# gvanhoy/gr-liquiddsp

Measured on AMD Instinct MI355X. Metric: Msamples/s through flex_rx (QPSK r1/2 1024B), higher is better.
Workload: dtype f32; 1 GPU; flex_rx single stream per GPU, 20000000 samples (10 Msym), PSK4 r=1/2 (CONV_V27), 1024-B payload, CRC-24, 256-sample gaps, CFO/phase/delay + AWGN Es/N0=20 dB; frames_decoded_ok=1154, streams_per_gpu=1, blocks_in_flight=12, stage_events=none (fxrx_set_timing level 0), steps=1415, passes=independent captures (reset between passes), segments=256, repairs=0

## Files before the change

gr-liquiddsp_amd/csrc/fx_host.cpp:

```cpp
#include <hip/hip_runtime.h>
#include <algorithm>
#include <chrono>
#include <cmath>
#include <cstdio>
#include <cstdlib>
#include <cstring>
#include <memory>
#include <string>
#include <vector>
#include "../../include/fxrx.h"
#include "fx_device.h"
#include "fx_codec.hpp"
#include "fx_launch.h"
#include "fx_traffic.h"

namespace {

thread_local std::string g_err;
void set_err(const std::string &s) { g_err = s; }

#define HIP_OK(expr)                                                                          \
    do {                                                                                      \
        hipError_t e_ = (expr);                                                               \
        if (e_ != hipSuccess) {                                                               \
            set_err(std::string(#expr) + ": " + hipGetErrorString(e_));                       \
            return FXRX_ERR_HIP;                                                              \
        }                                                                                     \
    } while (0)

template <class T> struct DevBuf {
    T *p = nullptr; size_t cap = 0;
    int reserve(size_t n)
    {
        if (n <= cap) return 0;
        size_t nc = std::max(n, cap + cap / 2);
        if (p) (void)hipFree(p);
        p = nullptr; cap = 0;
        if (hipMalloc((void **)&p, nc * sizeof(T)) != hipSuccess) { set_err("hipMalloc failed"); return FXRX_ERR_HIP; }
        cap = nc; return 0;
    }
    ~DevBuf() { if (p) (void)hipFree(p); }
};
template <class T> struct PinBuf {
    T *p = nullptr; size_t cap = 0;
    int reserve(size_t n)
    {
        if (n <= cap) return 0;
        size_t nc = std::max(n, cap + cap / 2);
        if (p) (void)hipHostFree(p);
        p = nullptr; cap = 0;
        if (hipHostMalloc((void **)&p, nc * sizeof(T), hipHostMallocDefault) != hipSuccess) { set_err("hipHostMalloc failed"); return FXRX_ERR_HIP; }
        cap = nc; return 0;
    }
    int grow_keep(size_t n, size_t keep)
    {
        if (n <= cap) return 0;
        T *np = nullptr;
        if (hipHostMalloc((void **)&np, n * sizeof(T), hipHostMallocDefault) != hipSuccess) { set_err("hipHostMalloc failed"); return FXRX_ERR_HIP; }
        if (p) { std::memcpy(np, p, std::min(keep, cap) * sizeof(T)); (void)hipHostFree(p); }
        p = np; cap = n; return 0;
    }
    ~PinBuf() { if (p) (void)hipHostFree(p); }
};

constexpr size_t kUploadKernelMax = 64u << 20;
static bool pinned_device_ptr(const void *p, const void **dev, uintptr_t align_mask = 7u)
{
    if (!p || (reinterpret_cast<uintptr_t>(p) & align_mask)) return false;
    hipPointerAttribute_t a;
    if (hipPointerGetAttributes(&a, p) != hipSuccess) { (void)hipGetLastError(); return false; }
    if (a.type != hipMemoryTypeHost || !a.devicePointer) return false;
    *dev = a.devicePointer;
    return true;
}
inline unsigned iq_sample_bytes(int fmt) { return fmt == FXRX_IQ_FC32 ? 8u : fmt == FXRX_IQ_SC16 ? 4u : fmt == FXRX_IQ_SC8 ? 2u : 0u; }
constexpr unsigned kMaxDepth = 32;
constexpr unsigned kStateRing = kMaxDepth + 3;
constexpr uint32_t kRepairCap = 256;

struct StreamState {
    float2 *carry[3] = { nullptr, nullptr, nullptr };
    int64_t carry_cap = 0;
    int64_t total = 0;
    bool fresh_start = true;
    int64_t carry_bound = 0;
    unsigned noskip_left = 0;
};

struct IngestJob { unsigned stream = 0; const void *dev_src = nullptr; const void *host_src = nullptr; uint64_t n = 0; };

struct StreamSnap { int64_t tot0 = 0; bool fresh_start = true; int64_t carry_bound = 0; bool noskip = false; };

}

struct Out { fxrx_frame f; };

enum StageEv { kEvStart = 0, kEvWalk, kEvVerify, kEvChain, kEvPlan, kEvMf, kEvPll, kEvDec, kEvDone, kEvHandover, kEvCount };
enum DecList { kDecPlain = 0, kDecRs, kDecBatch, kDecFallback, kDecLists };

struct Slot {
    hipStream_t st = nullptr;
    hipEvent_t ev[kEvCount] = {};
    unsigned index = 0;
    bool busy = false;
    uint64_t seq = 0;
    std::vector<const float2 *> x; std::vector<uint64_t> n; std::vector<StreamSnap> snap;
    std::vector<DevBuf<float2>> d_in;
    std::vector<DevBuf<uint8_t>> d_raw;
    std::vector<IngestJob> ingest; int ingest_fmt = FXRX_IQ_FC32; float ingest_scale = 0.0f;
    PinBuf<uint8_t> hp_desc; DevBuf<uint8_t> d_desc;
    size_t NJ = 0, n_early = 0, n_late = 0, o_list = 0, o_streams = 0;
    DevBuf<FxWalkResult> d_wres; DevBuf<FxFrame> d_frames, d_chain; DevBuf<FxVerifyRun> d_runs;
    DevBuf<FxBlockHdr> d_hdr;
    DevBuf<uint32_t> d_chain_count, d_stream_base, d_mf_job, d_mf_c0, d_pll_list, d_dec_list, d_vb_items;
    DevBuf<uint32_t> d_plan_ws;
    DevBuf<uint32_t> d_req;
    DevBuf<uint32_t> d_prescan;
    uint32_t ps_jobs = 0, ps_words = 0, ps_hops = 0, ps_taken = 0, ps_fallback = 0;
    DevBuf<uint32_t> d_cstat;
    DevBuf<uint8_t> d_vb_vec;
    DevBuf<unsigned long long> d_vb_dw;
    DevBuf<uint32_t> d_vb_st;
    uint32_t vb_cap = 0, vb_blk = 0;
    uint64_t vb_dw_words = 0, vb_slots_alloc = 128;
    DevBuf<FxPayJob> d_pjobs; DevBuf<FxPayResult> d_pres;
    uint32_t run_cap = 0, chain_cap = 0, mf_cap = 0, frame_slots = 0;
    uint64_t sym_cap = 0, byte_cap = 0, dw_cap = 0, out_cap = 0;
    DevBuf<float2> d_symraw;
    DevBuf<uint8_t> d_hard, d_bufA, d_bufB, d_soft; DevBuf<unsigned long long> d_dw;
    PinBuf<FxBlockHdr> h_hdr; PinBuf<FxOutRec> h_recs; PinBuf<uint8_t> h_out, h_soft; PinBuf<float2> h_framesyms;
    PinBuf<float2> h_win, h_wintail; PinBuf<uint32_t> h_winflag; uint32_t win_reserved = 0;
    std::vector<Out> out;
    uint64_t n_syms = 0;
    fxrx_timing timing{};
    double host_submit_ms = 0.0;
    bool any_late = false;
    double dbg_submit_ms = 0.0, dbg_collect_ms = 0.0, dbg_gpu_start_ms = 0.0, dbg_gpu_done_ms = 0.0;
    bool force_noskip = false;
    int timing_level = 0;
    bool inchain = false;
    uint32_t kept_hops = 0, kept_cheap = 0, kept_vhops = 0, kept_vfail = 0, kept_repairs = 0;
    TailPlan tail;
    bool tail_launched = true;
    hipStream_t tail_st = nullptr;
    uint32_t list_cap() const { return chain_cap + 64 * FX_PLL_CLASSES; }
    uint32_t *dec_list(DecList which) const { return d_dec_list.p + (size_t)which * list_cap(); }
    FxBlockHdr *hdr_walk() const { return d_hdr.p; } FxBlockHdr *hdr_pay() const { return d_hdr.p + 1; }
    const FxWalkJob *jobs() const { return reinterpret_cast<const FxWalkJob *>(d_desc.p); } FxWalkJob *jobs_rw() const { return reinterpret_cast<FxWalkJob *>(d_desc.p); }
    const uint32_t *job_list() const { return reinterpret_cast<const uint32_t *>(d_desc.p + o_list); } const FxStreamDesc *streams() const { return reinterpret_cast<const FxStreamDesc *>(d_desc.p + o_streams); }
#ifdef FX_STAMPS
    FxPayResult *pres() const { return d_pres.p; }
#else
    FxPayResult *pres() const { return nullptr; }
#endif
};

struct fxrx_ctx_s {
    fxrx_config cfg{};
    FxTables *d_tables = nullptr;
    std::vector<StreamState> st;
    FxStreamState *d_state = nullptr; FxStreamState *h_state = nullptr;
    float taper = -1.0f;
    bool skip_seek = true;
    bool chain_slow = false;
    unsigned pll_waves = 1, dec_waves = 1;
    int n_cus = 256;
    uint64_t seq = 0;
    hipEvent_t prev_chain = nullptr;
    hipEvent_t carry_reader[3] = { nullptr, nullptr, nullptr };
    Traffic traffic;
    bool batch_viterbi = true;
    bool vb_clean = true;
    int inchain_repair = 1; unsigned inchain_left = 0;
    bool plan_fused = true;
    bool vb_early_tail = true;
    int timing_level = -1;
    hipEvent_t ref_event = nullptr; double ref_host_ms = 0.0;
    int debug_walk_twice = 0;
    int debug_stop_after = 0;
    uint32_t walk_per_cu = 2;
    hipStream_t st_chain = nullptr;
    uint32_t verify_per_cu = 4;
    uint32_t mf_per_cu = 0;
    uint32_t plan_grid = 0;
    uint32_t vb_debug = 0, vb_blk_force = 0;
    std::vector<std::unique_ptr<Slot>> slots; unsigned depth = 1, head = 0, tail = 0, inflight = 0;
    Slot *last = nullptr;
    uint64_t replays = 0, repairs_host = 0, late_decodes = 0;
    uint64_t late_reason[6] = {};
    uint64_t late_windows = 0;
    uint32_t detwin_reserve = 0;
    unsigned noskip_left = 0;
    unsigned debug_fail_submit = 0, debug_fail_collect = 0;
    uint64_t discarded = 0;
    size_t ingest_kernel_max = 1u << 20;
    float iq_scale[3] = { 1.0f, 1.0f / 32768.0f, 1.0f / 128.0f };
    unsigned tail_gang = 4;
    bool prescan = false; int prescan_hops = -1;
    std::vector<Slot *> gang;
    uint64_t gang_launches = 0, gang_members = 0;
};

namespace {

std::unique_ptr<FxTables> make_tables()
{
    const fx::HostTables &H = fx::host_tables();
    const fx::BlockCodes &B = fx::block_codes();
    std::unique_ptr<FxTables> t(new FxTables);
    std::memset(t.get(), 0, sizeof(FxTables));
    for (int i = 0; i < 512; i++) { t->tw[i] = make_float2(H.tw[i].re, H.tw[i].im); t->S[i] = make_float2(H.S[i].re, H.S[i].im); }
    for (int i = 0; i < 1024; i++) t->sc[i] = make_float2(H.sc[i].re, H.sc[i].im);
    for (int i = 0; i < FX_S_LEN; i++) t->s[i] = make_float2(H.s[i].re, H.s[i].im);
    for (int i = 0; i < FX_HDR_PILOTS; i++) t->pilots[i] = make_float2(H.pilots[i].re, H.pilots[i].im);
    for (int i = 0; i < FX_PN_LEN; i++) t->pn[i] = make_float2(H.pn[i].re, H.pn[i].im);
    fx::design_eq_init(t->eq0);
    std::memcpy(t->proto, H.proto, sizeof H.proto);
    t->s2sum = H.s2sum;
    {
        fx::cf td[512]; std::memset(td, 0, sizeof td);
        float e = 0.0f, mr = 0.0f, mi = 0.0f;
        const int nd = FX_S_LEN - 1;
        for (int k = 0; k < nd; k++) {
            td[k].re = H.s[k + 1].re * H.s[k].re + H.s[k + 1].im * H.s[k].im;
            td[k].im = H.s[k + 1].im * H.s[k].re - H.s[k + 1].re * H.s[k].im;
            mr += td[k].re; mi += td[k].im;
        }
        mr /= (float)nd; mi /= (float)nd;
        for (int k = 0; k < nd; k++) { td[k].re -= mr; td[k].im -= mi; e += td[k].re * td[k].re + td[k].im * td[k].im; }
        fx::cf TD[512]; fx::hfft::fft512(td, TD, H.tw);
        for (int i = 0; i < 512; i++) t->TD[i] = make_float2(TD[i].re, TD[i].im);
        t->td2sum = e;
    }
    for (size_t i = 0; i < H.perm54.size(); i++) t->perm54[i] = (uint16_t)H.perm54[i];
    for (size_t i = 0; i < H.perm27.size(); i++) t->perm27[i] = (uint16_t)H.perm27[i];
    std::memcpy(t->h84dec, B.h84_dec, 256); std::memcpy(t->h84enc, B.h84_enc, 16); std::memcpy(t->sdcol, B.sd_col, 64);
    std::memcpy(t->sd22col, B.sd22_col, 16); std::memcpy(t->sd39col, B.sd39_col, 32);
    std::memcpy(t->h74dec, B.h74_dec, 128); std::memcpy(t->h128dec, B.h128_dec, 4096);
    std::memcpy(t->golenc, B.gol_enc, sizeof B.gol_enc); std::memcpy(t->golerr, B.gol_err, sizeof B.gol_err);
    std::memcpy(t->rsexp, B.rs_exp, 512); std::memcpy(t->rslog, B.rs_log, 256);
    for (int d = 0; d < 16; d++) t->h74enc[d] = B.h74_enc[d];
    for (int d = 0; d < 256; d++) t->h128enc[d] = B.h128_enc[d];
    {
        const uint8_t *cols[3] = { B.sd22_col, B.sd39_col, B.sd_col };
        const unsigned ncol[3] = { 16, 32, 64 };
        for (int c = 0; c < 3; c++) for (unsigned j = 0; j < ncol[c]; j++) t->sdinv[c][cols[c][j]] = (uint8_t)(j + 1);
    }
    return t;
}

int upload_tables(fxrx_ctx_s *c)
{
    std::unique_ptr<FxTables> t = make_tables();
    HIP_OK(hipMalloc((void **)&c->d_tables, sizeof(FxTables)));
    HIP_OK(hipMemcpy(c->d_tables, t.get(), sizeof(FxTables), hipMemcpyHostToDevice));
    return 0;
}

inline uint32_t seg_frames_cap(uint64_t seg, bool detect) { return (uint32_t)std::min<uint64_t>(seg / (detect ? 256 : 600) + 8, 4000); }

int alloc_carry(StreamState &S, int64_t cap)
{
    for (auto &p : S.carry) {
        if (p) (void)hipFree(p);
        p = nullptr;
        if (hipMalloc((void **)&p, (size_t)cap * sizeof(float2)) != hipSuccess) { set_err("hipMalloc (carry buffer) failed"); return FXRX_ERR_HIP; }
    }
    S.carry_cap = cap;
    return 0;
}

bool is_block_fec(unsigned fec)
{
    return fec == FX_FEC_HAMMING74 || fec == FX_FEC_HAMMING84 || fec == FX_FEC_HAMMING128 || fec == FX_FEC_GOLAY2412 ||
           fec == FX_FEC_SECDED2216 || fec == FX_FEC_SECDED3932 || fec == FX_FEC_SECDED7264;
}

constexpr unsigned kDebugMaxN = 1u << 18;

template <class Launch>
int debug_decode(const char *who, const uint8_t *in, size_t in_bytes, size_t in_pad, void *out, size_t out_bytes, void *out2, size_t out2_bytes,
                        Launch launch)
{
    int nd = 0;
    if (hipGetDeviceCount(&nd) != hipSuccess || nd <= 0) { set_err(std::string(who) + ": no usable HIP device"); return FXRX_ERR_NODEVICE; }
    std::unique_ptr<FxTables> t = make_tables();
    FxTables *d_t = nullptr; uint8_t *d_in = nullptr, *d_out = nullptr, *d_out2 = nullptr;
    auto run = [&]() -> int {
        HIP_OK(hipMalloc((void **)&d_t, sizeof(FxTables)));
        HIP_OK(hipMalloc((void **)&d_in, in_bytes + in_pad));
        HIP_OK(hipMalloc((void **)&d_out, out_bytes));
        if (out2) HIP_OK(hipMalloc((void **)&d_out2, out2_bytes));
        HIP_OK(hipMemcpy(d_t, t.get(), sizeof(FxTables), hipMemcpyHostToDevice));
        HIP_OK(hipMemcpy(d_in, in, in_bytes, hipMemcpyHostToDevice));
        HIP_OK(launch(d_in, d_out, d_out2, d_t));
        HIP_OK(hipDeviceSynchronize());
        HIP_OK(hipMemcpy(out, d_out, out_bytes, hipMemcpyDeviceToHost));
        if (out2) HIP_OK(hipMemcpy(out2, d_out2, out2_bytes, hipMemcpyDeviceToHost));
        return 0;
    };
    const int rc = run();
    for (void *p : { (void *)d_t, (void *)d_in, (void *)d_out, (void *)d_out2 }) if (p) (void)hipFree(p);
    return rc;
}

}

__attribute__((constructor)) static void fxrx_default_hw_queues() { setenv("GPU_MAX_HW_QUEUES", "16", 0); }

extern "C" {

const char *fxrx_last_error(void) { return g_err.c_str(); }
void fxrx_set_error(const char *msg) { set_err(msg ? msg : ""); }
const char *fxrx_version(void) { return "fxrx 0.2 (gfx950)"; }
int fxrx_device_count(void) { int n = 0; if (hipGetDeviceCount(&n) != hipSuccess) return 0; return n; }
void *fxrx_pinned_alloc(size_t bytes)
{
    void *p = nullptr;
    if (hipHostMalloc(&p, bytes ? bytes : 1, hipHostMallocDefault) != hipSuccess) { set_err("fxrx_pinned_alloc: hipHostMalloc failed"); return nullptr; }
    return p;
}
void fxrx_pinned_free(void *p) { if (p) (void)hipHostFree(p); }

static int make_slot(fxrx_ctx_s *c)
{
    std::unique_ptr<Slot> s(new Slot);
    HIP_OK(hipStreamCreateWithFlags(&s->st, hipStreamNonBlocking));
    for (auto &e : s->ev) HIP_OK(hipEventCreate(&e));
    s->index = (unsigned)c->slots.size();
    if (s->h_hdr.reserve(1) || s->d_hdr.reserve(2)) return FXRX_ERR_HIP;
    std::memset(s->h_hdr.p, 0, sizeof(FxBlockHdr));
    HIP_OK(hipMemset(s->d_hdr.p, 0, 2 * sizeof(FxBlockHdr)));
    c->slots.push_back(std::move(s));
    return 0;
}

static int close_gang(fxrx_ctx_s *c);
static void sync_all(fxrx_ctx_s *c) { if (c->st_chain) (void)hipStreamSynchronize(c->st_chain); for (auto &s : c->slots) if (s->st) (void)hipStreamSynchronize(s->st); }

static double g_prof[8]; static unsigned long g_prof_n;
static const bool g_prof_on = std::getenv("FXRX_DEBUG_SUBMIT_PROFILE") != nullptr;
static inline double prof_now() { return std::chrono::duration<double, std::milli>(std::chrono::steady_clock::now().time_since_epoch()).count(); }
void fxrx_destroy(fxrx_ctx *c)
{
    if (!c) return;
    (void)hipSetDevice(c->cfg.device);
    (void)close_gang(c);
    sync_all(c);
    if (g_prof_on && g_prof_n) {
        std::fprintf(stderr, "[fxrx] submit profile over %lu blocks (ms per block): upload + bookkeeping %.4f, segments %.4f, memory + descriptors %.4f, front launches %.4f, back launches %.4f\n",
                     g_prof_n, g_prof[0] / g_prof_n, g_prof[1] / g_prof_n, g_prof[2] / g_prof_n, g_prof[3] / g_prof_n, g_prof[4] / g_prof_n);
        for (auto &v : g_prof) v = 0.0; g_prof_n = 0;
    }
    for (auto &s : c->slots) {
        for (auto e : s->ev) if (e) (void)hipEventDestroy(e);
        if (s->st) (void)hipStreamDestroy(s->st);
    }
    if (c->st_chain) { (void)hipStreamSynchronize(c->st_chain); (void)hipStreamDestroy(c->st_chain); }
    for (auto &S : c->st) for (auto &p : S.carry) if (p) (void)hipFree(p);
    if (c->d_tables) (void)hipFree(c->d_tables);
    if (c->d_state) (void)hipFree(c->d_state);
    if (c->h_state) (void)hipHostFree(c->h_state);
    delete c;
}

fxrx_ctx *fxrx_create(const fxrx_config *cfg)
{
    if (!cfg || cfg->n_streams == 0) { set_err("fxrx_create: bad config"); return nullptr; }
    if (cfg->mode == FXRX_MODE_DETECTOR && cfg->soft_header) { set_err("fxrx_create: soft_header needs flex_rx mode (FXRX_ERR_ARG)"); return nullptr; }
    if (cfg->soft_block && (cfg->mode == FXRX_MODE_DETECTOR || !cfg->soft_decision)) {
        set_err("fxrx_create: soft_block needs soft_decision and flex_rx mode (FXRX_ERR_ARG)"); return nullptr;
    }
    if (cfg->soft_chain && (cfg->mode == FXRX_MODE_DETECTOR || !cfg->soft_decision || !cfg->soft_block)) {
        set_err("fxrx_create: soft_chain needs soft_block, soft_decision and flex_rx mode (FXRX_ERR_ARG)"); return nullptr;
    }
    if (cfg->soft_rs && (cfg->mode == FXRX_MODE_DETECTOR || !cfg->soft_decision)) {
        set_err("fxrx_create: soft_rs needs soft_decision and flex_rx mode (FXRX_ERR_ARG)"); return nullptr;
    }
    int nd = 0;
    if (hipGetDeviceCount(&nd) != hipSuccess || nd <= 0 || cfg->device >= nd) {
        set_err("fxrx_create: no usable HIP device (this library has no CPU path)"); return nullptr;
    }
    if (hipSetDevice(cfg->device) != hipSuccess) { set_err("hipSetDevice failed"); return nullptr; }
    fxrx_ctx_s *c = new fxrx_ctx_s;
    auto fail = [&]() -> fxrx_ctx * { const std::string keep = g_err; fxrx_destroy(c); set_err(keep); return nullptr; };
    c->cfg = *cfg;
    if (c->cfg.threshold <= 0.0f) c->cfg.threshold = cfg->mode == FXRX_MODE_DETECTOR ? 0.45f : 0.5f;
    if (const char *e = std::getenv("FXRX_PLL_WAVES")) c->pll_waves = (unsigned)std::min(4, std::max(1, std::atoi(e)));
    if (const char *e = std::getenv("FXRX_DEC_WAVES")) c->dec_waves = (unsigned)std::min(8, std::max(1, std::atoi(e)));
    if (const char *e = std::getenv("FXRX_SKIP_SEEK")) c->skip_seek = std::atoi(e) != 0;
    if (const char *e = std::getenv("FXRX_TAPER")) c->taper = std::min(0.95f, (float)std::atof(e));
    if (const char *e = std::getenv("FXRX_CHAIN_SLOW")) c->chain_slow = std::atoi(e) != 0;
    if (const char *e = std::getenv("FXRX_BATCH_VITERBI")) c->batch_viterbi = std::atoi(e) != 0;
    if (const char *e = std::getenv("FXRX_VB_CLEAN")) c->vb_clean = std::atoi(e) != 0;
    if (const char *e = std::getenv("FXRX_INCHAIN_REPAIR")) c->inchain_repair = std::min(2, std::max(0, std::atoi(e)));
    if (const char *e = std::getenv("FXRX_PLAN_FUSED")) c->plan_fused = std::atoi(e) != 0;
    if (const char *e = std::getenv("FXRX_VB_EARLY_TAIL")) c->vb_early_tail = std::atoi(e) != 0;
    if (const char *e = std::getenv("FXRX_DEBUG_STOP_AFTER")) c->debug_stop_after = std::atoi(e);
    if (const char *e = std::getenv("FXRX_DEBUG_WALK_TWICE")) c->debug_walk_twice = std::atoi(e);
    if (const char *e = std::getenv("FXRX_TIMING")) c->timing_level = std::min(2, std::max(0, std::atoi(e)));
    if (const char *e = std::getenv("FXRX_WALK_PER_CU")) c->walk_per_cu = (uint32_t)std::min(8, std::max(1, std::atoi(e)));
    if (const char *e = std::getenv("FXRX_VERIFY_PER_CU")) c->verify_per_cu = (uint32_t)std::min(64, std::max(1, std::atoi(e)));
    if (const char *e = std::getenv("FXRX_MF_PER_CU")) c->mf_per_cu = (uint32_t)std::min(64, std::max(0, std::atoi(e)));
    if (const char *e = std::getenv("FXRX_INGEST_KERNEL_MAX")) c->ingest_kernel_max = (size_t)std::max<long long>(0, std::atoll(e));
    if (const char *e = std::getenv("FXRX_PLAN_GRID")) c->plan_grid = (uint32_t)std::min(256, std::max(0, std::atoi(e)));
    if (const char *e = std::getenv("FXRX_DETWIN_RESERVE")) c->detwin_reserve = (uint32_t)std::max(0, std::atoi(e));
    if (const char *e = std::getenv("FXRX_VB_DEBUG")) c->vb_debug = (uint32_t)std::atoi(e);
    if (const char *e = std::getenv("FXRX_PRESCAN")) c->prescan = std::atoi(e) != 0;
    if (const char *e = std::getenv("FXRX_PRESCAN_HOPS")) c->prescan_hops = std::min<int>(FX_PRESCAN_MAX_HOPS, std::max(0, std::atoi(e)));
    if (const char *e = std::getenv("FXRX_TAIL_GANG")) c->tail_gang = (unsigned)std::min(FX_GANG_MAX, std::max(1, std::atoi(e)));
    if (const char *e = std::getenv("FXRX_VB_BLK")) if (std::atoi(e) > 0) c->vb_blk_force = (uint32_t)std::min(4096, std::max(128, (std::atoi(e) + 63) / 64 * 64));
    hipDeviceProp_t prop;
    if (hipGetDeviceProperties(&prop, cfg->device) == hipSuccess) c->n_cus = prop.multiProcessorCount;
    if (const char *e = std::getenv("FXRX_DEBUG_CUS")) c->n_cus = std::min(c->n_cus, std::max(1, std::atoi(e)));
    if (upload_tables(c) != 0) return fail();
    const unsigned NS = cfg->n_streams;
    c->st.resize(NS);
    int64_t cap0 = std::max<int64_t>(1 << 15, std::min<int64_t>(1 << 18, (int64_t)(1 << 24) / (int64_t)NS));
    if (const char *e = std::getenv("FXRX_CARRY_SAMPLES")) cap0 = std::max<int64_t>(1024, std::atoll(e));
    for (auto &S : c->st) if (alloc_carry(S, cap0) != 0) return fail();
    if (hipMalloc((void **)&c->d_state, sizeof(FxStreamState) * kStateRing * NS) != hipSuccess ||
        hipHostMalloc((void **)&c->h_state, sizeof(FxStreamState) * kStateRing * NS, hipHostMallocDefault) != hipSuccess) { set_err("fxrx_create: state ring allocation failed"); return fail(); }
    if (hipMemset(c->d_state, 0, sizeof(FxStreamState) * kStateRing * NS) != hipSuccess) { set_err("hipMemset failed"); return fail(); }
    std::memset(c->h_state, 0, sizeof(FxStreamState) * kStateRing * NS);
    for (unsigned i = 0; i < 2; i++) if (make_slot(c) != 0) return fail();
    return c;
}

void fxrx_reset(fxrx_ctx *c)
{
    if (!c) return;
    for (auto &S : c->st) { S.total = 0; S.fresh_start = true; S.carry_bound = 0; }
}

int fxrx_set_depth(fxrx_ctx *c, unsigned int depth)
{
    if (!c || depth == 0 || depth > kMaxDepth) return FXRX_ERR_ARG;
    HIP_OK(hipSetDevice(c->cfg.device));
    { const int r = close_gang(c); if (r) return r; }
    if (c->inflight) { set_err("fxrx_set_depth: blocks in flight"); return FXRX_ERR_STATE; }
    while (c->slots.size() < depth + 1) if (make_slot(c) != 0) return FXRX_ERR_HIP;
    c->depth = depth; c->head = c->tail = 0; c->last = nullptr;
    return 0;
}

int fxrx_debug_block_times(const fxrx_ctx *c, double out[4])
{
    if (!c || !c->last || !out) return FXRX_ERR_ARG;
    out[0] = c->last->dbg_submit_ms; out[1] = c->last->dbg_gpu_start_ms; out[2] = c->last->dbg_gpu_done_ms; out[3] = c->last->dbg_collect_ms;
    return 0;
}

int fxrx_set_timing(fxrx_ctx *c, int level)
{
    if (!c || level < -1 || level > 2) return FXRX_ERR_ARG;
    c->timing_level = level;
    if (!c->gang.empty()) { HIP_OK(hipSetDevice(c->cfg.device)); return close_gang(c); }
    return 0;
}

void *fxrx_stream(const fxrx_ctx *c) { return (c && !c->slots.empty()) ? (void *)c->slots[0]->st : nullptr; }

int fxrx_last_timing(const fxrx_ctx *c, fxrx_timing *t) { if (!c || !t || !c->last) return FXRX_ERR_ARG; *t = c->last->timing; return 0; }

const void *fxrx_device_framesyms(const fxrx_ctx *c, uint64_t *n)
{
    if (!c || !c->last) return nullptr;
    if (n) *n = c->last->n_syms;
    return c->last->n_syms ? c->last->d_symraw.p : nullptr;
}

enum WalkForm { kWalkList, kWalkRequests, kWalkRequestsInChain };
static inline hipError_t launch_walk(const fxrx_ctx_s *c, const Slot &sl, hipStream_t st, const uint32_t *list, unsigned njobs, WalkForm form = kWalkList)
{
    return fx_launch_walk(c->cfg.mode == FXRX_MODE_DETECTOR ? FX_MODE_DETECT : FX_MODE_FLEXRX, c->cfg.equalizer ? 1 : 0, c->cfg.soft_header ? 1 : 0, njobs, st, sl.jobs(), list, sl.d_wres.p, sl.d_frames.p, sl.d_runs.p,
                          sl.run_cap, sl.hdr_walk(), c->d_tables, form == kWalkList ? 0 : 1, (uint32_t)sl.NJ, form == kWalkRequestsInChain ? &sl.hdr_walk()->n_repair_req : nullptr, form == kWalkRequestsInChain ? (uint32_t)(2 * sl.NJ + 16) : 0u);
}
static inline hipError_t launch_seekverify(const fxrx_ctx_s *c, const Slot &sl, hipStream_t st, unsigned grid, uint32_t phase)
{
    return fx_launch_seekverify(grid, st, sl.d_runs.p, sl.run_cap, sl.jobs(), sl.d_wres.p, sl.d_frames.p, sl.hdr_walk(), c->d_tables, phase);
}
enum ChainForm { kStitch, kStitchQueue, kStitchPass1, kStitchPass2 };
static inline hipError_t launch_chainfast(const fxrx_ctx_s *c, const Slot &sl, hipStream_t st, ChainForm form)
{
    const bool queue = form == kStitchQueue || form == kStitchPass1;
    return fx_launch_chainfast(c->cfg.n_streams, st, sl.streams(), sl.jobs(), sl.d_wres.p, sl.d_frames.p, sl.d_chain.p, sl.d_chain_count.p, sl.hdr_walk(), form == kStitch && c->chain_slow ? 1u : 0u,
                               queue ? sl.jobs_rw() : nullptr, queue ? sl.d_req.p : nullptr, form >= kStitchPass1 ? sl.d_cstat.p : nullptr, form == kStitchPass1 ? 1u : form == kStitchPass2 ? 2u : 0u);
}
static inline int soft_level(const fxrx_config &cfg) { return cfg.soft_decision ? (cfg.soft_block ? (cfg.soft_chain ? 3 : 2) : 1) : 0; }
static inline hipError_t launch_paydec(const fxrx_ctx_s *c, const Slot &sl, hipStream_t st, DecList which, unsigned first_wave, unsigned n_waves, unsigned waves_per_wg)
{
    return fx_launch_paydec(which == kDecRs ? 1 : 0, which == kDecFallback ? 0 : soft_level(c->cfg), c->cfg.soft_rs ? 1 : 0, first_wave, n_waves, waves_per_wg, st, sl.d_pjobs.p, sl.dec_list(which), sl.hdr_pay(), sl.d_hard.p, sl.d_bufA.p, sl.d_bufB.p,
                            sl.d_soft.p, sl.d_dw.p, sl.h_out.p, sl.h_recs.p, sl.pres(), c->d_tables, which == kDecFallback ? sl.h_hdr.p : nullptr);
}
static inline hipError_t launch_decoders(const fxrx_ctx_s *c, const Slot &sl, hipStream_t st, unsigned first_plain, unsigned n_plain, unsigned n_rs)
{
    const hipError_t e = launch_paydec(c, sl, st, kDecPlain, first_plain, n_plain, c->dec_waves);
    return e != hipSuccess ? e : launch_paydec(c, sl, st, kDecRs, 0u, n_rs, 1u);
}
static inline hipError_t launch_trellis(const fxrx_ctx_s *c, const Slot &sl, hipStream_t st, unsigned n_items, int packed, int with_fix, unsigned n_fin, unsigned fb_waves)
{
    hipError_t e = fx_launch_vbitems(0, n_items, st, sl.d_pjobs.p, sl.d_vb_items.p, sl.vb_cap, sl.hdr_pay(), sl.d_bufA.p, sl.d_bufB.p, sl.d_vb_dw.p, sl.d_vb_vec.p, sl.d_vb_st.p, c->vb_debug, packed, with_fix);
    if (e == hipSuccess) e = fx_launch_vbfinish(0, n_fin, st, sl.d_pjobs.p, sl.dec_list(kDecBatch), sl.hdr_pay(), sl.d_bufA.p, sl.d_bufB.p, sl.d_vb_dw.p, sl.d_vb_vec.p, sl.d_vb_st.p, sl.dec_list(kDecFallback),
                                                sl.list_cap(), sl.h_out.p, sl.h_recs.p, sl.h_hdr.p, sl.tail.vb_early ? 1 : 0);
    return e != hipSuccess ? e : launch_paydec(c, sl, st, kDecFallback, 0u, fb_waves, 1u);
}
static inline hipError_t launch_detwin(const fxrx_ctx_s *c, const Slot &sl, uint32_t first, uint32_t last, bool late)
{
    return fx_launch_detwin(sl.st, std::min<unsigned>(std::max<unsigned>(last - first, 1u), 4u * (unsigned)c->n_cus), sl.streams(), c->cfg.n_streams, sl.d_stream_base.p, sl.d_pjobs.p, sl.hdr_pay(), first, last,
                            sl.h_win.p, sl.h_wintail.p, sl.h_winflag.p, late ? 0 : 1, late ? 1 : 0);
}
static void mark_noskip(fxrx_ctx_s *c, const Slot &sl, const std::vector<uint32_t> &req)
{
    const FxWalkJob *hj = reinterpret_cast<const FxWalkJob *>(sl.hp_desc.p);
    for (uint32_t r : req) if ((r & 0x80000000u) && (r & 0x7fffffffu) < sl.NJ) c->st[hj[r & 0x7fffffffu].stream].noskip_left = 32;
}

enum { kChainFast = 0, kChainFull = 1, kChainDone = 2 };
static int enqueue_back(fxrx_ctx_s *c, Slot &sl, int chain_mode, hipStream_t chain_st = nullptr, bool may_defer = false);

static int enqueue_block(fxrx_ctx_s *c, Slot &sl, bool may_defer = false)
{
    const unsigned NS = c->cfg.n_streams;
    const bool detect = c->cfg.mode == FXRX_MODE_DETECTOR;
    const uint64_t b = sl.seq;
    hipStream_t st = sl.st;
    const double tp0 = g_prof_on ? prof_now() : 0.0;

    uint32_t ps_K = 0;
    if (c->prescan && !detect) {
        if (c->prescan_hops >= 0) ps_K = (uint32_t)c->prescan_hops;
        else {
            ps_K = c->traffic.frames ? (uint32_t)std::min<uint64_t>(128, std::max<uint64_t>(16, c->traffic.samples / c->traffic.frames / FX_HOP + 2)) : 64u;
            ps_K = (ps_K + FX_PRESCAN_CHUNK - 1) / FX_PRESCAN_CHUNK * FX_PRESCAN_CHUNK;
        }
    }

    uint64_t seg = c->cfg.segment_len;
    if (seg == 0) {
        uint64_t tot = 0;
        for (unsigned s = 0; s < NS; s++) tot += sl.n[s];
        const uint64_t slots = (uint64_t)c->n_cus * c->walk_per_cu;
        if (c->depth > 1 && !detect) seg = tot / std::max<uint64_t>(std::max<uint64_t>(1, c->n_cus), std::min<uint64_t>(slots, 6 * slots / c->depth));
        else if (tot / slots < 131072) seg = tot / (slots - slots / 16);
        else seg = std::max<uint64_t>(tot / (4 * slots), 65536);
        seg = std::max<uint64_t>(seg, 32768); seg = std::min<uint64_t>(seg, 1u << 20);
    }
    seg = std::max<uint64_t>(seg, 4096);
    float taper = c->taper;
    if (taper < 0.0f) {
        uint64_t tot = 0;
        for (unsigned s = 0; s < NS; s++) tot += sl.n[s];
        taper = (detect && tot / seg > 4ull * (uint64_t)c->n_cus) ? 0.75f : 0.0f;
    }
    std::vector<FxWalkJob> jobs; std::vector<uint32_t> early, late; std::vector<FxStreamDesc> sds(NS);
    uint32_t frame_slots = 0, chain_slots = 0; uint64_t n_total = 0, carry_total = 0;
    for (unsigned s = 0; s < NS; s++) {
        StreamState &S = c->st[s]; const StreamSnap &sn = sl.snap[s];
        const int64_t ns = (int64_t)sl.n[s];
        const bool cont = !sn.fresh_start;
        FxStreamDesc &sd = sds[s];
        sd.x = sl.x[s]; sd.xa_end = cont ? S.carry[b % 3] + S.carry_cap : nullptr; sd.n = ns;
        sd.first_job = (uint32_t)jobs.size();
        sd.state_in = cont ? c->d_state + ((b + kStateRing - 1) % kStateRing) * NS + s : nullptr;
        sd.state_out = c->d_state + (b % kStateRing) * NS + s;
        sd.state_out_host = c->h_state + (b % kStateRing) * NS + s;
        sd.carry_out_end = S.carry[(b + 1) % 3] + S.carry_cap; sd.carry_cap = S.carry_cap;
        sd.abs_base = sn.tot0;
        int64_t p = 0; bool first = true;
        const int64_t seg0 = cont ? (int64_t)std::min<uint64_t>(seg, 8192) : (int64_t)seg;
        const int64_t p_t = cont ? std::min<int64_t>(ns, seg0) : 0;
        const int64_t k_t = taper > 0.0f ? std::max<int64_t>(1, ((ns - p_t) + (int64_t)seg / 2) / (int64_t)seg) : 0;
        int64_t i_t = 0;
        while (first || p < ns) {
            FxWalkJob j{};
            j.x = sd.x; j.xa_end = sd.xa_end; j.n = ns; j.start = p;
            j.stop = std::min<int64_t>(ns, p + (first ? seg0 : (int64_t)seg));
            if (ns - j.stop < (int64_t)seg / 2) j.stop = ns;
            if (k_t > 1 && p >= p_t) {
                const double u = (double)(i_t + 1) / (double)k_t;
                const int64_t e = p_t + (int64_t)((double)(ns - p_t) * (u * (1.0 + taper) - taper * u * u));
                j.stop = (i_t + 1 >= k_t) ? ns : std::min<int64_t>(ns, std::max<int64_t>(p + 4096, e & ~(int64_t)255));
                i_t++;
            }
            j.fresh = 1u; j.floor = p;
            j.mode = detect ? FX_MODE_DETECT : FX_MODE_FLEXRX;
            j.handoff = j.stop < ns ? 1u : 0u;
            j.prelock = first ? 0u : 1u;
            j.frame_base = frame_slots; j.max_frames = seg_frames_cap((uint64_t)(j.stop - j.start) + (first && cont ? (uint64_t)sn.carry_bound : 0u), detect);
            frame_slots += j.max_frames;
            j.threshold = c->cfg.threshold;
            j.no_skip = (detect || !c->skip_seek || sl.force_noskip || sn.noskip) ? 1u : 0u;
            j.state_in = (first && cont) ? sd.state_in : nullptr;
            j.stream = s; j.verify_per = c->traffic.verify_per; j.eq = (!detect && c->cfg.equalizer) ? 1u : 0u;
            (first && cont ? late : early).push_back((uint32_t)jobs.size());
            jobs.push_back(j);
            p = j.stop; first = false;
            if (p >= ns) break;
        }
        sd.n_jobs = (uint32_t)jobs.size() - sd.first_job;
        sd.chain_base = chain_slots; sd.chain_cap = (uint32_t)((uint64_t)(ns + (cont ? sn.carry_bound : 0)) / (detect ? 256u : 600u) + 8u);
        chain_slots += sd.chain_cap;
        n_total += (uint64_t)ns; carry_total += cont ? (uint64_t)sn.carry_bound : 0u;
    }
    for (unsigned s = 0; s < NS; s++) { sds[s].repair_base = frame_slots; sds[s].repair_cap = kRepairCap; frame_slots += kRepairCap; }
    if (taper > 0.0f)
        std::stable_sort(early.begin(), early.end(), [&](uint32_t a, uint32_t b2) { return jobs[a].stop - jobs[a].start > jobs[b2].stop - jobs[b2].start; });
    const size_t NJ = jobs.size();
    sl.NJ = NJ; sl.n_early = early.size(); sl.n_late = late.size(); sl.any_late = !late.empty();
    sl.frame_slots = frame_slots; sl.chain_cap = chain_slots;
    sl.run_cap = (uint32_t)std::min<uint64_t>((n_total + carry_total) / FX_HOP + 2 * NJ + 1024, 0x7fffffffu);
    const uint64_t span = n_total + carry_total;
    sl.sym_cap = span / 2 + 8ull * chain_slots + 64;
    sl.byte_cap = (span / 2) * 3 / 4 + 48ull * chain_slots + 64;
    sl.dw_cap = detect ? 0 : (span / 2) * 6 + 200ull * chain_slots + 64;
    sl.out_cap = (span / 2) * 3 / 4 + 16ull * chain_slots + 64;
    sl.mf_cap = (uint32_t)std::min<uint64_t>(span / 2 / 1024 + chain_slots + 16, 0x7fffffffu);
    {
        const uint64_t want_items = 64ull * 4ull * (uint64_t)c->n_cus * 6ull;
        sl.vb_blk = (detect || c->cfg.soft_decision || !c->batch_viterbi) ? 0u
                  : (uint32_t)std::min<uint64_t>(4096, std::max<uint64_t>(192, ((c->traffic.vb_steps / want_items + 63) / 64) * 64));
    }
    if (sl.vb_blk && c->vb_blk_force) sl.vb_blk = c->vb_blk_force;
    {
        const uint64_t steps_cap = std::min<uint64_t>(std::max<uint64_t>(span + span / 2, c->traffic.vb_steps + c->traffic.vb_steps / 4), 4 * span);
        sl.vb_cap = sl.vb_blk ? (uint32_t)((steps_cap / sl.vb_blk + 2048 + 127) & ~127ull) : 128u;
        sl.vb_dw_words = sl.vb_blk ? std::max<uint64_t>((uint64_t)sl.vb_cap * sl.vb_blk, steps_cap + 2176ull * 4096ull) : 0;
        sl.vb_slots_alloc = sl.vb_blk ? std::max<uint64_t>(sl.vb_cap, steps_cap / 192 + 2176) : 128;
    }
    if (sl.sym_cap >= (1ull << 32) || sl.dw_cap >= (1ull << 32)) { set_err("fxrx_submit: batch too large for 32-bit arena offsets"); return FXRX_ERR_ARG; }

    const double tp1 = g_prof_on ? prof_now() : 0.0;
    auto up16 = [](size_t v) { return (v + 15) & ~(size_t)15; };
    const size_t o_list = up16(NJ * sizeof(FxWalkJob)), o_streams = o_list + up16(2 * NJ * sizeof(uint32_t)), desc_bytes = o_streams + up16(NS * sizeof(FxStreamDesc));
    sl.o_list = o_list; sl.o_streams = o_streams;
    std::vector<uint32_t> spec;
    if (ps_K) for (uint32_t ji : early) if (jobs[ji].prelock && jobs[ji].mode == FX_MODE_FLEXRX) spec.push_back(ji);
    sl.ps_jobs = (uint32_t)spec.size(); sl.ps_hops = ps_K; sl.ps_words = (ps_K + FX_PRESCAN_CHUNK - 1) / FX_PRESCAN_CHUNK; sl.ps_taken = sl.ps_fallback = 0;
    if (!spec.empty()) {
        if (sl.d_prescan.reserve(spec.size() * sl.ps_words)) return FXRX_ERR_HIP;
        for (size_t i = 0; i < spec.size(); i++) {
            FxWalkJob &j = jobs[spec[i]];
            j.prescan = sl.d_prescan.p + i * sl.ps_words; j.prescan_words = sl.ps_words;
            j.prescan_hops = fx_prescan_valid_hops(j.start, j.stop, j.n, ps_K);
        }
    }
    if (sl.hp_desc.reserve(desc_bytes) || sl.d_desc.reserve(desc_bytes) || sl.d_wres.reserve(NJ + NS) || sl.d_frames.reserve(frame_slots) ||
        sl.d_runs.reserve(sl.run_cap) || sl.d_req.reserve(2 * NJ + 16) || sl.d_cstat.reserve(NS) || sl.d_chain.reserve(chain_slots) || sl.d_chain_count.reserve(NS) || sl.d_stream_base.reserve(NS + 1) ||
        sl.d_pjobs.reserve(chain_slots) || sl.h_recs.reserve(chain_slots) || sl.d_mf_job.reserve(sl.mf_cap) || sl.d_mf_c0.reserve(sl.mf_cap) ||
        sl.d_pll_list.reserve(sl.list_cap()) || sl.d_dec_list.reserve(kDecLists * (size_t)sl.list_cap())) return FXRX_ERR_HIP;
    if (!detect && (sl.d_symraw.reserve(sl.sym_cap) || sl.d_hard.reserve(sl.sym_cap + 64) ||
                    sl.d_bufA.reserve(sl.byte_cap + 256) || sl.d_bufB.reserve(sl.byte_cap + 256) || sl.d_dw.reserve(sl.dw_cap) || sl.h_out.reserve(sl.out_cap))) return FXRX_ERR_HIP;
    if (!detect && c->cfg.want_framesyms && sl.h_framesyms.reserve(sl.sym_cap)) return FXRX_ERR_HIP;
    if (detect && c->cfg.want_framesyms) {
        sl.win_reserved = c->detwin_reserve ? std::min(chain_slots, c->detwin_reserve) : with_margin(c->traffic.frames, chain_slots);
        if (sl.h_win.reserve((size_t)sl.win_reserved * FX_NFFT) || sl.h_wintail.reserve(2 * (size_t)NS * FX_NFFT) || sl.h_winflag.reserve(1)) return FXRX_ERR_HIP;
        *sl.h_winflag.p = 0u;
    }
    if (!sl.d_plan_ws.p) {
        if (sl.d_plan_ws.reserve(fx_plan_ws_words())) return FXRX_ERR_HIP;
        HIP_OK(hipMemsetAsync(sl.d_plan_ws.p, 0, fx_plan_ws_words() * sizeof(uint32_t), st));
    }
    if (sl.d_vb_items.reserve(2 * (size_t)sl.vb_slots_alloc) ||
        (sl.vb_blk && (sl.d_vb_vec.reserve(128 * (size_t)sl.vb_slots_alloc) || sl.d_vb_dw.reserve((size_t)sl.vb_dw_words) || sl.d_vb_st.reserve(sl.vb_slots_alloc)))) return FXRX_ERR_HIP;
    if (!detect && c->cfg.soft_decision && (sl.d_soft.reserve(8 * sl.byte_cap) || (c->cfg.want_framesyms && sl.h_soft.reserve(8 * sl.byte_cap)))) return FXRX_ERR_HIP;
#ifdef FX_STAMPS
    if (!detect && sl.d_pres.reserve(chain_slots)) return FXRX_ERR_HIP;
#endif
    std::memcpy(sl.hp_desc.p, jobs.data(), NJ * sizeof(FxWalkJob));
    uint32_t *hl = reinterpret_cast<uint32_t *>(sl.hp_desc.p + o_list);
    if (!early.empty()) std::memcpy(hl, early.data(), early.size() * sizeof(uint32_t));
    if (!late.empty()) std::memcpy(hl + early.size(), late.data(), late.size() * sizeof(uint32_t));
    if (!spec.empty()) std::memcpy(hl + NJ, spec.data(), spec.size() * sizeof(uint32_t));
    std::memcpy(sl.hp_desc.p + o_streams, sds.data(), NS * sizeof(FxStreamDesc));
    const uint32_t *d_list = sl.job_list();

    const double tp2 = g_prof_on ? prof_now() : 0.0;
    if (!sl.ingest.empty()) {
        std::vector<IngestJob> todo; todo.swap(sl.ingest);
        const size_t bytes = iq_sample_bytes(sl.ingest_fmt);
        for (const IngestJob &j : todo) {
            const void *src = j.dev_src;
            if (!src) { HIP_OK(hipMemcpyAsync(sl.d_raw[j.stream].p, j.host_src, j.n * bytes, hipMemcpyHostToDevice, st)); src = sl.d_raw[j.stream].p; }
            HIP_OK(fx_launch_ingest(st, sl.ingest_fmt, src, sl.d_in[j.stream].p, (size_t)j.n, sl.ingest_scale, (unsigned)c->n_cus));
        }
    }
    HIP_OK(fx_launch_upload(st, sl.hp_desc.p, sl.d_desc.p, desc_bytes, (unsigned)c->n_cus));
    const int tl = c->timing_level >= 0 ? c->timing_level : (c->depth > 1 ? 0 : 2);
    sl.timing_level = tl;
    if (c->debug_walk_twice > 0) HIP_OK(fx_launch_prescan(st, (unsigned)spec.size(), sl.ps_words, sl.jobs(), d_list + NJ, c->d_tables));
    for (int rep = 0; rep < c->debug_walk_twice; rep++) HIP_OK(launch_walk(c, sl, st, d_list, (unsigned)early.size()));
    if (tl >= 2) HIP_OK(hipEventRecord(sl.ev[kEvStart], st));
    if (c->debug_walk_twice <= 0) HIP_OK(fx_launch_prescan(st, (unsigned)spec.size(), sl.ps_words, sl.jobs(), d_list + NJ, c->d_tables));
    HIP_OK(launch_walk(c, sl, st, d_list, (unsigned)early.size()));
    const bool verify = !detect && c->skip_seek && !sl.force_noskip;
    hipStream_t cst = st;
    if (!late.empty()) {
        if (verify) {
            HIP_OK(fx_launch_copy_u32(st, &sl.hdr_walk()->n_runs, &sl.hdr_walk()->runs_done));
            HIP_OK(launch_seekverify(c, sl, st, c->verify_per_cu * (unsigned)c->n_cus, 0u));
        }
        if (!c->st_chain) {
            int lo = 0, hi = 0;
            HIP_OK(hipDeviceGetStreamPriorityRange(&lo, &hi));
            HIP_OK(hipStreamCreateWithPriority(&c->st_chain, hipStreamNonBlocking, hi));
        }
        HIP_OK(hipEventRecord(sl.ev[kEvHandover], st));
        cst = c->st_chain;
        HIP_OK(hipStreamWaitEvent(cst, sl.ev[kEvHandover], 0));
        if (c->prev_chain) HIP_OK(hipStreamWaitEvent(cst, c->prev_chain, 0));
        HIP_OK(launch_walk(c, sl, cst, d_list + early.size(), (unsigned)late.size()));
    }
    if (tl >= 2) HIP_OK(hipEventRecord(sl.ev[kEvWalk], cst));
    if (verify)
        HIP_OK(launch_seekverify(c, sl, cst, late.empty() ? c->verify_per_cu * (unsigned)c->n_cus : (unsigned)std::min<size_t>((size_t)c->verify_per_cu * (size_t)c->n_cus, std::max<size_t>(64, 16 * late.size())), 1u));
    if (tl >= 2) HIP_OK(hipEventRecord(sl.ev[kEvVerify], cst));
    if (late.empty() && c->prev_chain) HIP_OK(hipStreamWaitEvent(cst, c->prev_chain, 0));
    if (c->carry_reader[(b + 1) % 3]) HIP_OK(hipStreamWaitEvent(cst, c->carry_reader[(b + 1) % 3], 0));
    const double tp3 = g_prof_on ? prof_now() : 0.0;
    const int rb = enqueue_back(c, sl, kChainFast, cst, may_defer);
    if (g_prof_on) { const double tp4 = prof_now(); g_prof[1] += tp1 - tp0; g_prof[2] += tp2 - tp1; g_prof[3] += tp3 - tp2; g_prof[4] += tp4 - tp3; g_prof_n++; }
    return rb;
}

static FxVbpreMember vbpre_member(Slot &sl, uint32_t first_wave, uint32_t n_waves)
{
    return FxVbpreMember{ sl.d_pjobs.p, sl.dec_list(kDecBatch), sl.hdr_pay(), sl.d_hard.p, sl.d_bufA.p, sl.d_bufB.p, sl.h_out.p, sl.h_recs.p, sl.h_hdr.p, first_wave, n_waves };
}
static int launch_tails(fxrx_ctx_s *c, Slot *const *m, unsigned n)
{
    hipStream_t st = m[n - 1]->st;
    for (unsigned i = 0; i + 1 < n; i++) HIP_OK(hipStreamWaitEvent(st, m[i]->ev[kEvMf], 0));
    auto done = [&]() -> int {
        for (unsigned i = 0; i < n; i++) { HIP_OK(hipEventRecord(m[i]->ev[kEvDone], st)); m[i]->tail_launched = true; m[i]->tail_st = st; }
        if (n > 1) { c->gang_launches++; c->gang_members += n; }
        return 0;
    };
    {
        FxPllGang g; unsigned waves[FX_GANG_MAX]; g.n = n;
        for (unsigned i = 0; i < n; i++) { const Slot &sl = *m[i]; g.m[i] = FxPllMember{ sl.d_pjobs.p, sl.d_pll_list.p, sl.hdr_pay(), sl.d_symraw.p, sl.d_symraw.p, sl.d_hard.p, sl.h_recs.p }; waves[i] = sl.tail.pll_waves; }
        HIP_OK(fx_launch_paypll(&g, waves, c->pll_waves, st, c->d_tables));
    }
    for (unsigned i = 0; i < n; i++) if (m[i]->timing_level >= 1) HIP_OK(hipEventRecord(m[i]->ev[kEvPll], st));
    if (c->debug_stop_after == 6) return done();
    for (unsigned i = 0; i < n; i++) {
        Slot &sl = *m[i];
        if (c->cfg.soft_decision) {
            HIP_OK(fx_launch_softdemod(sl.tail.mf_grid, st, sl.d_pjobs.p, sl.d_mf_job.p, sl.d_mf_c0.p, sl.hdr_pay(), sl.d_symraw.p, sl.d_hard.p, sl.d_soft.p, c->d_tables));
            if (c->cfg.want_framesyms) HIP_OK(hipMemcpyAsync(sl.h_soft.p, sl.d_soft.p, 8 * sl.byte_cap, hipMemcpyDeviceToHost, st));
        }
        HIP_OK(launch_decoders(c, sl, st, 0u, sl.tail.plain, sl.tail.rs));
    }
    {
        FxVbpreGang g; g.n = n;
        for (unsigned i = 0; i < n; i++) g.m[i] = vbpre_member(*m[i], 0u, m[i]->vb_blk ? m[i]->tail.vb_pre : 0u);
        HIP_OK(fx_launch_vbpre(&g, st, c->d_tables, c->vb_clean ? 1 : 0, c->vb_early_tail && c->vb_clean ? 1 : 0));
    }
    for (unsigned i = 0; i < n; i++) {
        Slot &sl = *m[i];
        if (sl.vb_blk) HIP_OK(launch_trellis(c, sl, st, sl.tail.vb_items, sl.tail.vb_packed, sl.tail.with_fix, sl.tail.vb_fin, sl.tail.fb));
        if (sl.timing_level >= 2) HIP_OK(hipEventRecord(sl.ev[kEvDec], st));
        if (c->cfg.want_framesyms) HIP_OK(fx_launch_symcopy(2u * (unsigned)c->n_cus, st, sl.hdr_pay(), sl.d_symraw.p, sl.h_framesyms.p));
    }
    return done();
}

static int close_gang(fxrx_ctx_s *c)
{
    if (c->gang.empty()) return 0;
    if (c->gang.size() > FX_GANG_MAX) { set_err("open gang larger than FX_GANG_MAX (internal error)"); return FXRX_ERR_STATE; }
    Slot *m[FX_GANG_MAX]; unsigned n = 0;
    for (Slot *s : c->gang) m[n++] = s;
    c->gang.clear();
    return launch_tails(c, m, n);
}

static int enqueue_back(fxrx_ctx_s *c, Slot &sl, int chain_mode, hipStream_t chain_st, bool may_defer)
{
    const unsigned NS = c->cfg.n_streams; const bool detect = c->cfg.mode == FXRX_MODE_DETECTOR;
    const uint64_t b = sl.seq; const uint32_t chain_slots = sl.chain_cap; hipStream_t st = sl.st;
    sl.tail_launched = true; sl.tail_st = st;
    if (chain_mode == kChainFull)
        HIP_OK(fx_launch_chain(detect ? FX_MODE_DETECT : FX_MODE_FLEXRX, c->cfg.equalizer ? 1 : 0, c->cfg.soft_header ? 1 : 0, NS, st, sl.streams(), sl.jobs(), (uint32_t)sl.NJ, sl.d_wres.p, sl.d_frames.p, sl.d_chain.p,
                               sl.d_chain_count.p, sl.d_runs.p, sl.run_cap, sl.hdr_walk(), c->chain_slow ? 1u : 0u, c->d_tables));
    else if (chain_mode == kChainFast) {
        hipStream_t cs = chain_st ? chain_st : st;
        sl.inchain = !c->chain_slow && (c->inchain_repair == 2 || (c->inchain_repair == 1 && c->inchain_left > 0));
        if (c->inchain_left) c->inchain_left--;
        if (!sl.inchain) HIP_OK(launch_chainfast(c, sl, cs, kStitch));
        else {
            HIP_OK(launch_chainfast(c, sl, cs, kStitchPass1));
            HIP_OK(launch_walk(c, sl, cs, sl.d_req.p, (unsigned)std::min<size_t>(2 * sl.NJ, 64), kWalkRequestsInChain));
            HIP_OK(launch_chainfast(c, sl, cs, kStitchPass2));
        }
    }
    HIP_OK(hipEventRecord(sl.ev[kEvChain], chain_mode == kChainFast && chain_st ? chain_st : st));
    if (chain_mode == kChainFast && chain_st && chain_st != st) HIP_OK(hipStreamWaitEvent(st, sl.ev[kEvChain], 0));
    c->prev_chain = sl.ev[kEvChain];
    {
        FxPlanArgs a;
        a.streams = sl.streams(); a.nstreams = NS; a.detect = detect ? 1u : 0u; a.eq = c->cfg.equalizer ? 1u : 0u; a.vb_blk = sl.vb_blk;
        a.chain = sl.d_chain.p; a.chain_count = sl.d_chain_count.p; a.stream_base = sl.d_stream_base.p;
        a.pjobs = sl.d_pjobs.p; a.recs = sl.h_recs.p;
        a.mf_job = sl.d_mf_job.p; a.mf_c0 = sl.d_mf_c0.p; a.mf_cap = sl.mf_cap;
        a.pll_list = sl.d_pll_list.p; a.dec_list = sl.dec_list(kDecPlain); a.list_cap = sl.list_cap();
        a.vb_items = sl.d_vb_items.p; a.vb_cap = sl.vb_cap;
        a.hdr = sl.hdr_walk(); a.hdr_pay = sl.hdr_pay(); a.hdr_host = sl.h_hdr.p; a.ws = sl.d_plan_ws.p;
        HIP_OK(fx_launch_plan(st, c->plan_grid ? c->plan_grid : (unsigned)std::min<uint64_t>(64, c->traffic.frames / 2048 + 1), c->plan_fused ? 1 : 0, a));
    }
    const int tl = sl.timing_level;
    if (tl >= 2) HIP_OK(hipEventRecord(sl.ev[kEvPlan], st));
    if (c->debug_stop_after == 4) { c->carry_reader[b % 3] = nullptr; HIP_OK(hipEventRecord(sl.ev[kEvDone], st)); return 0; }
    if (!detect) {
        const TailPlan plan = plan_tail(c->traffic, TailCaps{ chain_slots, sl.mf_cap, sl.vb_cap, sl.vb_blk }, TailKnobs{ c->depth, c->n_cus, c->mf_per_cu, c->vb_debug, c->vb_early_tail, c->vb_clean });
        HIP_OK(fx_launch_paymf(plan.mf_grid, c->cfg.equalizer ? 1 : 0, st, sl.d_pjobs.p, sl.d_mf_job.p, sl.d_mf_c0.p, sl.hdr_pay(), sl.d_chain.p, sl.d_symraw.p, c->d_tables));
        HIP_OK(hipEventRecord(sl.ev[kEvMf], st));
        c->carry_reader[b % 3] = sl.ev[kEvMf];
        if (c->debug_stop_after == 5) { HIP_OK(hipEventRecord(sl.ev[kEvDone], st)); return 0; }
        sl.tail = plan;
        if (sl.vb_blk && c->traffic.trellis_left) c->traffic.trellis_left--;
        sl.timing.trellis_launched = plan.vb_fin ? 1 : 0;
        unsigned ahead = 0;
        for (unsigned k = 0; k < c->inflight; k++) ahead += c->slots[(c->tail + k) % (c->depth + 1)]->tail_launched ? 1u : 0u;
        const unsigned G = c->tail_gang;
        if (G >= 2 && may_defer && c->depth >= 4 && c->traffic.seen && !c->debug_stop_after && tl <= 1 && ahead >= G) {
            sl.tail_launched = false; sl.tail_st = nullptr;
            c->gang.push_back(&sl);
            return c->gang.size() >= G ? close_gang(c) : 0;
        }
        { const int r = close_gang(c); if (r) return r; }
        Slot *one = &sl;
        return launch_tails(c, &one, 1u);
    } else {
        if (c->cfg.want_framesyms) HIP_OK(launch_detwin(c, sl, 0u, sl.win_reserved, false));
        HIP_OK(hipEventRecord(sl.ev[kEvMf], st));
        if (tl >= 1) HIP_OK(hipEventRecord(sl.ev[kEvPll], st));
        if (tl >= 2) HIP_OK(hipEventRecord(sl.ev[kEvDec], st));
        c->carry_reader[b % 3] = sl.ev[kEvMf];
    }
    HIP_OK(hipEventRecord(sl.ev[kEvDone], st));
    return 0;
}

static int prepare_ingest(fxrx_ctx_s *c, Slot &sl, const void *const *iq, const uint64_t *n_samples, int on_device, int fmt)
{
    const unsigned NS = c->cfg.n_streams;
    const size_t bytes = iq_sample_bytes(fmt);
    sl.ingest.clear();
    for (unsigned s = 0; s < NS; s++)
        if (n_samples[s] && (!iq[s] || (reinterpret_cast<uintptr_t>(iq[s]) & (bytes - 1)))) {
            set_err("fxrx_submit_fmt: integer IQ must be aligned to its sample size (sc16: 4 bytes, sc8: 2 bytes)"); return FXRX_ERR_ARG;
        }
    if (sl.d_in.size() < NS) sl.d_in.resize(NS);
    if (sl.d_raw.size() < NS) sl.d_raw.resize(NS);
    std::vector<IngestJob> jobs;
    for (unsigned s = 0; s < NS; s++) {
        const uint64_t nn = n_samples[s];
        if (sl.d_in[s].reserve(nn + 1)) return FXRX_ERR_HIP;
        if (!nn) continue;
        IngestJob j; j.stream = s; j.n = nn;
        if (on_device) j.dev_src = iq[s];
        else if (!(nn * bytes <= c->ingest_kernel_max && pinned_device_ptr(iq[s], &j.dev_src, 0u))) {
            j.dev_src = nullptr; j.host_src = iq[s];
            if (sl.d_raw[s].reserve(nn * bytes + 16)) return FXRX_ERR_HIP;
        }
        jobs.push_back(j);
    }
    sl.ingest.swap(jobs); sl.ingest_fmt = fmt; sl.ingest_scale = c->iq_scale[fmt];
    return 0;
}

static int submit_block(fxrx_ctx *c, const void *const *iq, const uint64_t *n_samples, int on_device, int fmt)
{
    if (!c || !iq || !n_samples) { set_err("fxrx_submit: null argument"); return FXRX_ERR_ARG; }
    if (iq_sample_bytes(fmt) == 0) { set_err("fxrx_submit_fmt: unknown IQ format"); return FXRX_ERR_ARG; }
    if (c->inflight >= c->depth) { set_err("fxrx_submit: pipeline full, call fxrx_collect first"); return FXRX_ERR_STATE; }
    HIP_OK(hipSetDevice(c->cfg.device));
    const auto t_enter = std::chrono::steady_clock::now();
    const unsigned NS = c->cfg.n_streams;
    const unsigned nslots = c->depth + 1;
    Slot &sl = *c->slots[c->head];
    sl.ingest.clear();
    if (fmt != FXRX_IQ_FC32) { const int r = prepare_ingest(c, sl, iq, n_samples, on_device, fmt); if (r) return r; }
    sl.out.clear(); sl.timing = fxrx_timing{};
    sl.kept_hops = sl.kept_cheap = sl.kept_vhops = sl.kept_vfail = sl.kept_repairs = 0;
    const unsigned noskip_before = c->noskip_left;
    sl.force_noskip = c->noskip_left > 0; if (c->noskip_left) c->noskip_left--;
    sl.seq = c->seq;
    sl.x.assign(NS, nullptr); sl.n.assign(n_samples, n_samples + NS); sl.snap.assign(NS, StreamSnap{});
    if (sl.d_in.size() < NS) sl.d_in.resize(NS);
    struct Undo { fxrx_ctx_s *c; std::vector<StreamState> st; unsigned noskip; bool armed = true;
                  ~Undo() { if (armed) { c->st = st; c->noskip_left = noskip; } } } undo{ c, c->st, noskip_before };
    uint64_t total_new = 0;
    for (unsigned s = 0; s < NS; s++) {
        StreamState &S = c->st[s];
        const uint64_t nn = n_samples[s];
        total_new += nn;
        if (fmt != FXRX_IQ_FC32) sl.x[s] = sl.d_in[s].p;
        else if (on_device) sl.x[s] = (const float2 *)iq[s];
        else {
            if (sl.d_in[s].reserve(nn + 1)) return FXRX_ERR_HIP;
            if (nn) {
                const void *dsrc = nullptr;
                if (nn * sizeof(float2) <= kUploadKernelMax && pinned_device_ptr(iq[s], &dsrc)) HIP_OK(fx_launch_upload(sl.st, dsrc, sl.d_in[s].p, nn * sizeof(float2), (unsigned)c->n_cus));
                else HIP_OK(hipMemcpyAsync(sl.d_in[s].p, iq[s], nn * sizeof(float2), hipMemcpyHostToDevice, sl.st));
            }
            sl.x[s] = sl.d_in[s].p;
        }
        sl.snap[s].tot0 = S.total; sl.snap[s].fresh_start = S.fresh_start; sl.snap[s].carry_bound = S.fresh_start ? 0 : S.carry_bound;
        sl.snap[s].noskip = S.noskip_left > 0; if (S.noskip_left) S.noskip_left--;
        S.total += (int64_t)nn; S.fresh_start = false;
        S.carry_bound = std::min<int64_t>(S.carry_cap, sl.snap[s].carry_bound + (int64_t)nn);
    }
    if (c->timing_level >= 2 && !c->ref_event) {
        if (hipEventCreate(&c->ref_event) == hipSuccess) { (void)hipEventRecord(c->ref_event, sl.st); (void)hipEventSynchronize(c->ref_event); c->ref_host_ms = std::chrono::duration<double, std::milli>(std::chrono::steady_clock::now().time_since_epoch()).count(); }
    }
    sl.dbg_submit_ms = std::chrono::duration<double, std::milli>(std::chrono::steady_clock::now().time_since_epoch()).count() - c->ref_host_ms;
    sl.timing.samples = total_new;
    if (c->debug_fail_submit) { c->debug_fail_submit--; set_err("fxrx_submit: injected failure (fxrx_debug_fail)"); return FXRX_ERR_STATE; }
    if (g_prof_on) g_prof[0] += prof_now() - std::chrono::duration<double, std::milli>(t_enter.time_since_epoch()).count();
    int r = enqueue_block(c, sl,  true);
    if (r) return r;
    undo.armed = false;
    c->seq++;
    sl.busy = true;
    c->head = (c->head + 1) % nslots; c->inflight++;
    sl.host_submit_ms = std::chrono::duration<double, std::milli>(std::chrono::steady_clock::now() - t_enter).count();
    return 0;
}

int fxrx_submit(fxrx_ctx *c, const void *const *iq, const uint64_t *n_samples, int on_device) { return submit_block(c, iq, n_samples, on_device, FXRX_IQ_FC32); }
int fxrx_submit_fmt(fxrx_ctx *c, const void *const *iq, const uint64_t *n_samples, int on_device, int fmt) { return submit_block(c, iq, n_samples, on_device, fmt); }

unsigned int fxrx_iq_sample_bytes(int fmt) { return iq_sample_bytes(fmt); }

int fxrx_set_iq_scale(fxrx_ctx *c, int fmt, float scale)
{
    if (!c || (fmt != FXRX_IQ_SC16 && fmt != FXRX_IQ_SC8) || !std::isfinite(scale) || !(scale > 0.0f)) { set_err("fxrx_set_iq_scale: bad argument"); return FXRX_ERR_ARG; }
    c->iq_scale[fmt] = scale;
    return 0;
}

int fxrx_iq_convert_host(int fmt, float scale, const void *in, uint64_t n_samples, float *out_re_im)
{
    if (iq_sample_bytes(fmt) == 0 || (n_samples && (!in || !out_re_im))) { set_err("fxrx_iq_convert_host: bad argument"); return FXRX_ERR_ARG; }
    const uint64_t nc = 2 * n_samples;
    if (fmt == FXRX_IQ_FC32) { if (nc) std::memcpy(out_re_im, in, nc * sizeof(float)); }
    else if (fmt == FXRX_IQ_SC16) { const int16_t *q = static_cast<const int16_t *>(in); for (uint64_t i = 0; i < nc; i++) out_re_im[i] = (float)q[i] * scale; }
    else { const int8_t *q = static_cast<const int8_t *>(in); for (uint64_t i = 0; i < nc; i++) out_re_im[i] = (float)q[i] * scale; }
    return 0;
}

static int repair_rounds(fxrx_ctx_s *c, Slot &sl)
{
    if (c->chain_slow) return 1;
    hipStream_t st = sl.st; FxBlockHdr *hdr = sl.hdr_walk();
    for (int round = 0; round < 64; round++) {
        HIP_OK(hipMemsetAsync(hdr, 0, sizeof(FxBlockHdr), st));
        HIP_OK(launch_chainfast(c, sl, st, kStitchQueue));
        FxBlockHdr hh;
        HIP_OK(hipMemcpyAsync(&hh, hdr, sizeof hh, hipMemcpyDeviceToHost, st));
        HIP_OK(hipStreamSynchronize(st));
        if (std::getenv("FXRX_DEBUG_ROUNDS")) std::fprintf(stderr, "[fxrx] repair round %d: flags %x requests %u\n", round, hh.flags, hh.n_repair_req);
        if (!(hh.flags & FX_BLK_NEEDS_REPAIR)) return 0;
        if ((hh.flags & FX_BLK_NEEDS_SLOW) || hh.n_repair_req == 0 || hh.n_repair_req > 2 * sl.NJ) break;
        {
            std::vector<uint32_t> req(hh.n_repair_req);
            HIP_OK(hipMemcpyAsync(req.data(), sl.d_req.p, req.size() * sizeof(uint32_t), hipMemcpyDeviceToHost, st));
            HIP_OK(hipStreamSynchronize(st));
            mark_noskip(c, sl, req);
        }
        HIP_OK(hipMemsetAsync(hdr, 0, sizeof(FxBlockHdr), st));
        HIP_OK(launch_walk(c, sl, st, sl.d_req.p, hh.n_repair_req, kWalkRequests));
        HIP_OK(hipMemcpyAsync(&hh, hdr, sizeof hh, hipMemcpyDeviceToHost, st));
        HIP_OK(hipStreamSynchronize(st));
        sl.kept_hops += hh.hops; sl.kept_cheap += hh.hops_cheap; sl.kept_repairs += hh.walk_jobs_run ? hh.walk_jobs_run : 0;
    }
    HIP_OK(hipMemsetAsync(hdr, 0, sizeof(FxBlockHdr), st));
    return 1;
}

static int repair_and_replay(fxrx_ctx_s *c, Slot &sl)
{
    const unsigned NS = c->cfg.n_streams;
    const unsigned nslots = c->depth + 1;
    unsigned n_dep = 0;
    for (unsigned k = 1; k < c->inflight; k++) {
        const Slot &nx = *c->slots[(c->tail + k) % nslots];
        bool dep = false;
        for (unsigned s = 0; s < NS; s++) dep = dep || !nx.snap[s].fresh_start;
        if (!dep) break;
        n_dep++;
    }
    const hipEvent_t newest_chain = c->prev_chain;
    bool carry_moved = false;
    { const int r = close_gang(c); if (r) return r; }
    for (int round = 0; round < 6; round++) {
        HIP_OK(hipStreamSynchronize(sl.st));
        for (unsigned k = 1; k <= n_dep; k++) {
            const Slot &nx = *c->slots[(c->tail + k) % nslots];
            HIP_OK(hipStreamSynchronize(nx.st));
            if (nx.tail_st && nx.tail_st != nx.st) HIP_OK(hipStreamSynchronize(nx.tail_st));
        }
        const uint32_t flags = sl.h_hdr.p->flags;
        if (std::getenv("FXRX_DEBUG_ROUNDS")) std::fprintf(stderr, "[fxrx] block %llu at collect: flags %x verify_failures %u (pass %d)\n", (unsigned long long)sl.seq, flags, sl.h_hdr.p->verify_failures, round);
        if (flags & FX_BLK_NEEDS_REPAIR) {
            c->repairs_host++; c->inchain_left = 16;
            const FxBlockHdr &h0 = *sl.h_hdr.p;
            sl.kept_hops += h0.hops; sl.kept_cheap += h0.hops_cheap; sl.kept_vhops += h0.verify_hops; sl.kept_vfail += h0.verify_failures;
            sl.ps_taken += h0.ps_taken; sl.ps_fallback += h0.ps_fallback;
            if (!sl.force_noskip && c->cfg.mode != FXRX_MODE_DETECTOR && c->skip_seek && h0.verify_failures > std::max<uint32_t>(16u, (uint32_t)sl.NJ / 8u)) {
                sl.force_noskip = true; c->noskip_left = 32;
                if (enqueue_block(c, sl)) return FXRX_ERR_HIP;
            } else {
                const int rr = repair_rounds(c, sl);
                if (rr < 0 || enqueue_back(c, sl, rr == 0 ? kChainDone : kChainFull)) return FXRX_ERR_HIP;
            }
            continue;
        }
        if (!(flags & FX_BLK_CARRY_OVERFLOW)) break;
        const uint64_t b = sl.seq;
        FxStreamState *hs = c->h_state + (b % kStateRing) * NS, *ds = c->d_state + (b % kStateRing) * NS;
        for (auto &o : c->slots) if (o->busy) HIP_OK(hipStreamSynchronize(o->st));
        carry_moved = true;
        for (unsigned s = 0; s < NS; s++) {
            if (!hs[s].overflow) continue;
            StreamState &S = c->st[s];
            const int64_t keep = hs[s].carry_len, old_cap = S.carry_cap;
            float2 *old[3] = { S.carry[0], S.carry[1], S.carry[2] };
            S.carry[0] = S.carry[1] = S.carry[2] = nullptr;
            int64_t cap = std::max<int64_t>(2 * old_cap, 2 * keep); cap = (cap + 4095) & ~(int64_t)4095;
            if (alloc_carry(S, cap)) return FXRX_ERR_HIP;
            const int64_t nb = (int64_t)sl.n[s], from = nb - keep;
            float2 *dst = S.carry[(b + 1) % 3] + cap - keep;
            if (from < 0) HIP_OK(hipMemcpy(dst, old[b % 3] + old_cap + from, (size_t)(-from) * sizeof(float2), hipMemcpyDeviceToDevice));
            const int64_t n_new = std::min<int64_t>(keep, nb);
            if (n_new > 0) HIP_OK(hipMemcpy(dst + (keep - n_new), sl.x[s] + (nb - n_new), (size_t)n_new * sizeof(float2), hipMemcpyDeviceToDevice));
            for (auto p : old) if (p) (void)hipFree(p);
            hs[s].overflow = 0; hs[s].invalid = 0;
            HIP_OK(hipMemcpy(ds + s, hs + s, sizeof(FxStreamState), hipMemcpyHostToDevice));
        }
        sl.h_hdr.p->flags &= ~(uint32_t)FX_BLK_CARRY_OVERFLOW;
        c->replays++;
        break;
    }
    if (sl.h_hdr.p->flags & (FX_BLK_NEEDS_REPAIR | FX_BLK_CARRY_OVERFLOW)) { set_err("fxrx_collect: block could not be repaired"); return FXRX_ERR_STATE; }
    if (sl.h_hdr.p->flags & FX_BLK_CHAIN_FULL) { set_err("fxrx_collect: chain table overflow (internal sizing error)"); return FXRX_ERR_STATE; }
    c->prev_chain = sl.ev[kEvChain];
    const unsigned n_replay = carry_moved ? c->inflight - 1 : n_dep;
    for (unsigned k = 1; k <= n_replay; k++) {
        Slot &nx = *c->slots[(c->tail + k) % nslots];
        for (unsigned s = 0; s < NS; s++) if (!nx.snap[s].fresh_start) nx.snap[s].carry_bound = c->st[s].carry_cap;
        int r = enqueue_block(c, nx);
        if (r) return r;
    }
    if (n_replay + 1 < c->inflight) c->prev_chain = newest_chain;
    for (auto &S : c->st) S.carry_bound = S.carry_cap;
    return 0;
}

static int finish_decode(fxrx_ctx_s *c, Slot &sl)
{
    FxBlockHdr *hdr_pay = sl.hdr_pay();
    auto fetch_fb = [&]() -> int { uint32_t nfb = 0; HIP_OK(hipMemcpy(&nfb, &hdr_pay->n_vb_fallback, sizeof nfb, hipMemcpyDeviceToHost)); sl.h_hdr.p->n_vb_fallback = nfb; sl.h_hdr.p->vb_ticket = 0; return 0; };
    if (sl.vb_blk && sl.h_hdr.p->vb_ticket && fetch_fb()) return FXRX_ERR_HIP;
    FxBlockHdr h = *sl.h_hdr.p; h.vb_dirty = *(volatile const uint32_t *)&sl.h_hdr.p->vb_dirty;
    TailPlan &p = sl.tail;
    const LateWork w = late_work(p, h, sl.vb_blk);
    if (!w.any()) return 0;
    HIP_OK(launch_decoders(c, sl, sl.st, p.plain, w.more_plain ? h.n_dec_plain - p.plain : 0u, w.more_rs ? h.n_dec_rs : 0u));
    if (w.more_batch() || w.late_trellis) {
        HIP_OK(hipMemsetAsync(&hdr_pay->n_vb_fallback, 0, sizeof(uint32_t), sl.st));
        if (w.more_batch()) {
            FxVbpreGang g; g.n = 1; g.m[0] = vbpre_member(sl, 0u, h.n_dec_batch);
            HIP_OK(fx_launch_vbpre(&g, sl.st, c->d_tables, c->vb_clean ? 1 : 0, p.vb_early ? 1 : 0));
        }
        HIP_OK(launch_trellis(c, sl, sl.st, h.n_vb_items, 1, 1, h.n_dec_batch, kFallbackWaves));
        p.vb_pre = p.vb_fin = h.n_dec_batch; p.vb_items = h.n_vb_items; p.fb = kFallbackWaves;
        HIP_OK(hipStreamSynchronize(sl.st));
        if (fetch_fb()) return FXRX_ERR_HIP;
    }
    const uint32_t n_fb = *(volatile const uint32_t *)&sl.h_hdr.p->n_vb_fallback;
    if (sl.vb_blk && n_fb > p.fb) {
        HIP_OK(launch_paydec(c, sl, sl.st, kDecFallback, p.fb, n_fb - p.fb, c->dec_waves));
        p.fb = n_fb;
    }
    HIP_OK(hipStreamSynchronize(sl.st));
    p.plain = std::max(p.plain, h.n_dec_plain); if (w.more_rs) p.rs = h.n_dec_rs;
    c->late_decodes++;
    w.count(c->late_reason);
    return 0;
}

static int finish_windows(fxrx_ctx_s *c, Slot &sl)
{
    if (*(volatile const uint32_t *)sl.h_winflag.p) { set_err("fxrx_collect: more than two detections of a stream start in its carried tail (internal sizing error)"); return FXRX_ERR_STATE; }
    const uint32_t n = sl.h_hdr.p->n_frames;
    if (n <= sl.win_reserved) return 0;
    { const int r = sl.h_win.grow_keep((size_t)n * FX_NFFT, (size_t)sl.win_reserved * FX_NFFT); if (r) return r; }
    HIP_OK(launch_detwin(c, sl, sl.win_reserved, n, true));
    HIP_OK(hipStreamSynchronize(sl.st));
    c->late_windows++;
    return 0;
}

static void discard_inflight(fxrx_ctx_s *c)
{
    const std::string keep = g_err;
    (void)close_gang(c);
    sync_all(c);
    const unsigned nslots = c->depth + 1;
// ... 291 lines not shown
```

gr-liquiddsp_amd/csrc/fx_kernels.hip:

```cpp
#include <hip/hip_runtime.h>
#include <algorithm>
#include "fx_device.h"
#include "fx_launch.h"
#include "fx_vbclean.h"
#include "fx_rsgmd.h"

#define HALF         256

template <int WW> struct WalkLdsT {
    static constexpr int WAVES = WW;
    static constexpr bool SWEEP_PAIRS = WW == 4;
    float2 win[FX_NFFT];
    float2 X[FX_NFFT];
    float2 S[FX_NFFT];
    float2 scr[WW][576];
    float2 v[640];
    float2 P[256];
    float  m2[FX_NFFT];
    float2 hdr[FX_HDR_SYM];
    float2 cw[(WW + 1) * FX_HOP + 8];
    __device__ __forceinline__ float2 *scr2(int wave) { return wave < 2 ? v + 576 * wave : cw + 576 * (wave - 2); }
    float2 pb[16];
    float2 eqw[16];
    float  taps[FX_MF_TAPS];
// ... 1368 lines not shown
            const bool spliced = (cm & 0x8000u) != 0, nothing = spliced && nf <= m;
            const bool term = j + 1 == nj || ex != FX_EXIT_STOP || !((inf >> 27) & 1u);
            bool problem = ((inf >> 29) & 1u) || ex == FX_EXIT_TABLE_FULL || ex == FX_EXIT_INVALID;
            if (!nothing && ((inf >> 28) & 1u) && !((inf >> 30) & 1u)) problem = true;
            if (problem) C.sh[5] = 1;
            if ((inf >> 30) & 1u) problem = true;
            if (req_list && j + 1 < nj && ex == FX_EXIT_STOP && !((inf >> 27) & 1u) && jobs[first + j].handoff) problem = true;
            if (!term && ((lk >> 11) & 4095u) == CHAIN_NONE) {
                problem = true;
                if (req_list) {
                    const uint32_t k = lk & 2047u; const FxWalkResult &R = results[first + j];
                    FxWalkJob &J = jobs_rw[first + k];
                    J.start = R.pos; J.floor = R.floor; J.fresh = R.fresh ? 1u : 0u; J.prelock = 0; J.no_skip = 1; J.state_in = nullptr; J.pad_ = 1;
                    req_list[atomicAdd(&hdr_rw->n_repair_req, 1u)] = first + k;
                }
            }
            if (problem) C.sh[0] = 1;
            const uint32_t pj = C.pred[j];
            const uint32_t contrib = j == 0 ? c0 : ((inf >> 12) & 4095u) - (pj == 0xFFFFu ? 0u : C.skip[pj]);
            const uint32_t upto = c0 + C.P[j];
            C.accA[j] = upto - contrib;
            if (term || problem) { C.sh[1] = j; C.sh[2] = nothing ? 1u : 0u; C.sh[3] = upto; }
        }
        __syncthreads();
        if (tid == 0 && !C.sh[0] && C.sh[3] > sd.chain_cap) { C.sh[0] = 1; C.sh[5] = 1; }
        __syncthreads();
    }
    if (hdr_rw && blockIdx.x == 0 && tid == 0) hdr_rw->stamp[5] = (uint32_t)(__builtin_readcyclecounter() - tph_);
    if (!C.sh[0]) {
        for (uint32_t j = tid; j < nj; j += NT) {
            const uint32_t cm = C.m[j];
            if (cm == 0xFFFFu) continue;
            const uint32_t m = cm & 0x7FFFu, nf = C.info[j] & 4095u; const bool spliced = (cm & 0x8000u) != 0;
            const FxFrame *F = frames + jobs[first + j].frame_base;
            uint32_t o = C.accA[j];
            for (uint32_t i = m; i < nf; i++) {
                const uint32_t fl = F[i].flags;
                if (!(fl & FX_FLAG_EXACT)) continue;
                const bool own = !(spliced && i == m);
                if (own && (fl & FX_FLAG_SPAN_BAD)) { C.sh[0] = 1; C.sh[5] = 1; }
                copy_frame(out + o, F + i);
                if (!own) out[o].rxy = results[first + C.pred[j]].handoff_rxy;
                o++;
            }
        }
    }
    __syncthreads();
    const bool ok = !C.sh[0];
    if (ok) {
        const uint32_t ej = C.sh[1];
        const FxWalkResult &R = C.sh[2] ? results[first + C.pred[ej]] : results[first + ej];
        fin_pos = R.pos; fin_floor = R.floor; fin_fresh = R.fresh != 0; cnt = C.sh[3];
    }
    __syncthreads();
    return ok;
}

template <int NT>
__device__ __forceinline__ void chain_finish(const FxStreamDesc &sd, uint32_t s, const FxStreamState &st_in, uint32_t cnt, int64_t fin_pos, int64_t fin_floor,
                                             bool fin_fresh, uint32_t *chain_count, FxBlockHdr *hdr)
{
    const int tid = threadIdx.x;
    const XSrc xs = make_xsrc(sd.x, sd.xa_end, sd.n);
    if (cnt > sd.chain_cap) { if (tid == 0) atomicOr(&hdr->flags, (uint32_t)FX_BLK_CHAIN_FULL); cnt = sd.chain_cap; }
    int64_t keep_from = fin_fresh ? fin_pos : fin_pos - FX_HOP;
    keep_from = max(-st_in.carry_len, min(keep_from, sd.n));
    const int64_t keep = sd.n - keep_from;
    const bool overflow = keep > sd.carry_cap;
    if (!overflow)
        for (int64_t i = tid; i < keep; i += NT) sd.carry_out_end[i - keep] = xld(xs, keep_from + i);
    if (tid == 0) {
        FxStreamState so;
        so.pos = fin_pos - sd.n; so.floor = max(fin_floor - sd.n, -keep); so.carry_len = keep; so.fresh = fin_fresh ? 1u : 0u;
        so.invalid = overflow ? 1u : 0u; so.overflow = overflow ? 1u : 0u; so.pad_ = 0;
        *sd.state_out = so; *sd.state_out_host = so;
        chain_count[s] = cnt;
        if (overflow) atomicOr(&hdr->flags, (uint32_t)FX_BLK_CARRY_OVERFLOW);
    }
}

__device__ __forceinline__ bool chain_state_in(const FxStreamDesc *streams, const FxStreamDesc &sd, uint32_t s, FxStreamState &st_in, uint32_t *chain_count, FxBlockHdr *hdr)
{
    st_in.pos = 0; st_in.floor = 0; st_in.carry_len = 0; st_in.fresh = 1; st_in.invalid = 0; st_in.overflow = 0; st_in.pad_ = 0;
    if (sd.state_in) st_in = *sd.state_in;
    int other = 0;
    for (uint32_t t = threadIdx.x; t < gridDim.x; t += blockDim.x) {
        const FxStreamState *p = streams[t].state_in;
        if (p && p->invalid) other = 1;
    }
    if (!__syncthreads_or(other) && !st_in.invalid) return true;
    if (threadIdx.x == 0) {
        FxStreamState so = st_in; so.invalid = 1; so.overflow = 0;
        *sd.state_out = so; *sd.state_out_host = so; chain_count[s] = 0;
        atomicOr(&hdr->flags, (uint32_t)FX_BLK_INVALID);
    }
    return false;
}

#define CHAINFAST_THREADS 256
extern "C" __global__ __launch_bounds__(CHAINFAST_THREADS)
void fx_chainfast_kernel(const FxStreamDesc *streams, const FxWalkJob *jobs, const FxWalkResult *results, const FxFrame *frames, FxFrame *chain,
                         uint32_t *chain_count, FxBlockHdr *hdr, uint32_t force_repair, FxWalkJob *jobs_rw, uint32_t *req_list, uint32_t *stat, uint32_t pass)
{
    __shared__ ChainLds C;
    const uint32_t s = blockIdx.x;
    if (pass == 2u && stat[s] != 2u) return;
    const FxStreamDesc sd = streams[s];
    FxStreamState st_in;
    if (!chain_state_in(streams, sd, s, st_in, chain_count, hdr)) { if (pass == 1u && threadIdx.x == 0) stat[s] = 3u; return; }
    uint32_t cnt = 0; int64_t fin_pos = 0, fin_floor = 0; bool fin_fresh = true;
    const unsigned long long t0_ = __builtin_readcyclecounter();
    if (threadIdx.x == 0) C.sh[5] = 0;
    __syncthreads();
    const bool ok = !force_repair && chain_fast_path<CHAINFAST_THREADS>(sd, jobs, results, frames, chain + sd.chain_base, C, cnt, fin_pos, fin_floor, fin_fresh,
                                                                        pass == 2u ? nullptr : jobs_rw, pass == 2u ? nullptr : req_list, hdr);
    if (s == 0 && threadIdx.x == 0) { hdr->stamp[0] = (uint32_t)(__builtin_readcyclecounter() - t0_); }
    if (!ok) {
        if (threadIdx.x == 0) {
            const bool slow = force_repair || sd.n_jobs > CHAIN_MAXJ || C.sh[5];
            if (pass == 1u && !slow) stat[s] = 2u;
            else {
                FxStreamState so = st_in; so.invalid = 1; so.overflow = 0;
                *sd.state_out = so; *sd.state_out_host = so; chain_count[s] = 0;
                atomicOr(&hdr->flags, (uint32_t)(FX_BLK_NEEDS_REPAIR | (slow ? FX_BLK_NEEDS_SLOW : 0)));
                if (pass) stat[s] = 3u;
            }
        }
        return;
    }
    if (pass && threadIdx.x == 0) stat[s] = 1u;
    chain_finish<CHAINFAST_THREADS>(sd, s, st_in, cnt, fin_pos, fin_floor, fin_fresh, chain_count, hdr);
    if (s == 0 && threadIdx.x == 0) hdr->stamp[3] = (uint32_t)(__builtin_readcyclecounter() - t0_);
}

extern "C" hipError_t fx_launch_chainfast(unsigned nstreams, hipStream_t st, const FxStreamDesc *streams, const FxWalkJob *jobs, const FxWalkResult *results,
                                          const FxFrame *frames, FxFrame *chain, uint32_t *chain_count, FxBlockHdr *hdr, uint32_t force_repair,
                                          FxWalkJob *jobs_rw, uint32_t *req_list, uint32_t *stat, uint32_t pass)
{
    hipLaunchKernelGGL(fx_chainfast_kernel, dim3(nstreams), dim3(CHAINFAST_THREADS), 0, st, streams, jobs, results, frames, chain, chain_count, hdr, force_repair,
                       jobs_rw, req_list, stat, pass);
    return hipGetLastError();
}

template <int MODE, int WW, bool EQ, bool SH>
__device__ __forceinline__ void chain_kernel_body(const FxStreamDesc *streams, const FxWalkJob *jobs, uint32_t n_jobs_total, FxWalkResult *results,
                                                  FxFrame *frames, FxFrame *chain, uint32_t *chain_count, FxVerifyRun *runs, uint32_t run_cap,
                                                  FxBlockHdr *hdr, uint32_t force_slow, const FxTables *T, typename WalkLdsSel<MODE, WW>::type &L, ChainLds &C)
{
    constexpr int NT = 64 * WW;
    const uint32_t s = blockIdx.x;
    const FxStreamDesc sd = streams[s];
    const int tid = threadIdx.x, lane = tid & 63;
    FxFrame *out = chain + sd.chain_base;
    FxStreamState st_in;
    if (!chain_state_in(streams, sd, s, st_in, chain_count, hdr)) return;
    float2 twA[7], twB[7];
#pragma unroll
    for (int r = 1; r < 8; r++) { twA[r - 1] = T->tw[lane * r]; twB[r - 1] = T->tw[8 * (lane & 7) * r]; }
    for (int i = tid; i < FX_NFFT; i += NT) L.S[i] = T->S[i];

    const uint32_t first = sd.first_job, end = first + sd.n_jobs;
    uint32_t cnt = 0;
    int64_t fin_pos = 0, fin_floor = 0; bool fin_fresh = true;
    bool done = !force_slow && chain_fast_path<NT>(sd, jobs, results, frames, out, C, cnt, fin_pos, fin_floor, fin_fresh);

    if (!done) {
        uint32_t cur = first, m = 0;
        const FxWalkResult *Rp = results + cur; const FxFrame *F = frames + jobs[cur].frame_base;
        FxWalkResult *rep_res = results + n_jobs_total + s;
        float splice_rxy = -1.0f; bool spliced = false;
        int64_t tpos = 0, tfloor = 0; bool tfresh = true;
        cnt = 0;
        bool need_walk = false; uint32_t wj = 0; int64_t wst = 0, wfl = 0; bool wfr = false;
        auto repair = [&](uint32_t jidx, int64_t st, int64_t fl, bool fr) { need_walk = true; wj = jidx; wst = st; wfl = fl; wfr = fr; };
        for (;;) {
            if (need_walk) {
                FxWalkJob j = jobs[wj];
                j.start = wst; j.floor = wfl; j.fresh = wfr ? 1u : 0u; j.prelock = 0; j.no_skip = 1; j.state_in = nullptr;
                j.frame_base = sd.repair_base; j.max_frames = sd.repair_cap;
                __syncthreads();
                walk_any<MODE, WW, EQ, false, SH>(j, wj, rep_res, frames, runs, run_cap, hdr, T, L, twA, twB);
                wg_sync_global();
                if (tid == 0) atomicAdd(&hdr->repairs, 1u);
                Rp = rep_res; F = frames + sd.repair_base; m = 0; need_walk = false;
            }
            const FxWalkResult R = *Rp;
            uint32_t nf = R.n_frames;
            if (R.exit_code == FX_EXIT_PAYLOAD && nf > 0) nf--;
            int bad = -1;
            for (uint32_t i = m; i < nf; i++) {
                const uint32_t fl = F[i].flags;
                if (!(fl & FX_FLAG_EXACT)) continue;
                const bool own = !(i == m && splice_rxy >= 0.0f);
                if (own && (fl & FX_FLAG_SPAN_BAD)) { bad = (int)i; break; }
                if (cnt < sd.chain_cap) {
                    const uint32_t *a = reinterpret_cast<const uint32_t *>(F + i); uint32_t *b = reinterpret_cast<uint32_t *>(out + cnt);
                    if (tid < (int)(sizeof(FxFrame) / 4))
                        b[tid] = (!own && tid == (int)(offsetof(FxFrameHead, rxy) / 4)) ? __builtin_bit_cast(uint32_t, splice_rxy) : a[tid];
                }
                cnt++;
            }
            if (bad >= 0) {
                const int64_t sp = F[bad].seek_pos, sf = F[bad].seek_floor; const bool sfr = (F[bad].flags & FX_FLAG_SEEK_FRESH) != 0;
                repair(cur, sp, sf, sfr); spliced = false; splice_rxy = -1.0f; continue;
            }
            if (!(spliced && nf <= m) && (R.tail_flags & FX_FLAG_SPAN_BAD)) {
                repair(cur, R.tail_pos, R.tail_floor, (R.tail_flags & FX_FLAG_SEEK_FRESH) != 0); spliced = false; splice_rxy = -1.0f; continue;
            }
            splice_rxy = -1.0f;
            const bool last = (cur + 1 == end);
            if (R.exit_code == FX_EXIT_TABLE_FULL) { repair(cur, R.pos, R.floor, R.fresh != 0); spliced = false; continue; }
            if (last || R.exit_code != FX_EXIT_STOP || !R.has_handoff) {
                if (spliced && nf <= m) { fin_pos = tpos; fin_floor = tfloor; fin_fresh = tfresh; }
                else { fin_pos = R.pos; fin_floor = R.floor; fin_fresh = R.fresh != 0; }
                break;
            }
            spliced = false;
            uint32_t nxt = cur + 1;
            while (nxt + 1 < end && R.handoff_start >= jobs[nxt].stop + FX_HOP) nxt++;
            const FxWalkResult *RNp = results + nxt; const FxFrame *FN = frames + jobs[nxt].frame_base;
            const uint32_t nfn = RNp->n_frames;
            uint32_t found = 0xFFFFFFFFu;
            for (uint32_t i = 0; R.handoff_clear && i < nfn; i++) {
                const uint32_t fl = FN[i].flags;
                if ((fl & FX_FLAG_EXACT) && (fl & FX_FLAG_FLOOR_CLEAR) && FN[i].start == R.handoff_start && FN[i].offset == R.handoff_offset) { found = i; break; }
            }
            if (found != 0xFFFFFFFFu) {
                splice_rxy = R.handoff_rxy; spliced = true; tpos = R.pos; tfloor = R.floor; tfresh = R.fresh != 0;
                cur = nxt; m = found; Rp = RNp; F = FN; continue;
            }
            repair(nxt, R.pos, R.floor, R.fresh != 0);
            cur = nxt;
        }
        __syncthreads();
    }

    chain_finish<NT>(sd, s, st_in, cnt, fin_pos, fin_floor, fin_fresh, chain_count, hdr);
}

template <int MODE, int WW, bool EQ, bool SH = false>
__global__ __launch_bounds__(64 * WW, 1)
void fx_chain_kernel(const FxStreamDesc *streams, const FxWalkJob *jobs, uint32_t n_jobs_total, FxWalkResult *results, FxFrame *frames,
                     FxFrame *chain, uint32_t *chain_count, FxVerifyRun *runs, uint32_t run_cap, FxBlockHdr *hdr, uint32_t force_slow,
                     const FxTables *T)
{
    static_assert(!SH || MODE == FX_MODE_FLEXRX, "soft header decoding is a flex_rx variant");
    __shared__ typename WalkLdsSel<MODE, WW>::type L;
    __shared__ ChainLds C;
    chain_kernel_body<MODE, WW, EQ, SH>(streams, jobs, n_jobs_total, results, frames, chain, chain_count, runs, run_cap, hdr, force_slow, T, L, C);
}

extern "C" hipError_t fx_launch_chain(unsigned mode, int eq, int sh, unsigned nstreams, hipStream_t st, const FxStreamDesc *streams, const FxWalkJob *jobs, uint32_t n_jobs_total,
                                      FxWalkResult *results, FxFrame *frames, FxFrame *chain, uint32_t *chain_count, FxVerifyRun *runs, uint32_t run_cap,
                                      FxBlockHdr *hdr, uint32_t force_slow, const FxTables *T)
{
#define FX_CHAIN_LAUNCH(M, W, E, S) hipLaunchKernelGGL((fx_chain_kernel<M, W, E, S>), dim3(nstreams), dim3(64 * W), 0, st, streams, jobs, n_jobs_total, results, frames, chain, chain_count, runs, run_cap, hdr, force_slow, T)
#define FX_CHAIN_FLEX(S) do { if (eq) FX_CHAIN_LAUNCH(FX_MODE_FLEXRX, FX_FLEX_WAVES, true, S); else FX_CHAIN_LAUNCH(FX_MODE_FLEXRX, FX_FLEX_WAVES, false, S); } while (0)
    if (mode == FX_MODE_DETECT) FX_CHAIN_LAUNCH(FX_MODE_DETECT, FX_DETECT_WAVES, false, false);
    else if (sh) FX_CHAIN_FLEX(true);
    else FX_CHAIN_FLEX(false);
#undef FX_CHAIN_FLEX
#undef FX_CHAIN_LAUNCH
    return hipGetLastError();
}

template <bool SOFT>
__global__ __launch_bounds__(64 * FX_FLEX_WAVES)
void fx_hdrdec_kernel(const uint8_t *in, uint32_t n, uint8_t *out, int32_t *valid, const FxTables *T)
{
    __shared__ WalkLdsT<FX_FLEX_WAVES> L;
    const int tid = threadIdx.x;
    for (uint32_t h = blockIdx.x; h < n; h += gridDim.x) {
        if constexpr (SOFT) { for (int i = tid; i < 8 * FX_HDR_ENC; i += 64 * FX_FLEX_WAVES) L.hsoft()[i] = in[(size_t)h * (8 * FX_HDR_ENC) + i]; }
        else if (tid < FX_HDR_ENC) L.b0[tid] = in[(size_t)h * FX_HDR_ENC + tid];
        __syncthreads();
        if constexpr (SOFT) decode_header_soft(L, T, tid); else decode_header_bytes(L, T, tid);
        if (tid < FX_HDR_DEC) out[(size_t)h * FX_HDR_DEC + tid] = L.b1[tid];
        if (tid == 0) valid[h] = (int32_t)L.u[1];
        __syncthreads();
    }
}
extern "C" hipError_t fx_launch_hdrdec(int soft, unsigned n, hipStream_t st, const uint8_t *in, uint8_t *out, int32_t *valid, const FxTables *T)
{
    if (n == 0) return hipSuccess;
    const unsigned grid = std::min(n, 65536u);
    if (soft) hipLaunchKernelGGL((fx_hdrdec_kernel<true>), dim3(grid), dim3(64 * FX_FLEX_WAVES), 0, st, in, n, out, valid, T);
    else hipLaunchKernelGGL((fx_hdrdec_kernel<false>), dim3(grid), dim3(64 * FX_FLEX_WAVES), 0, st, in, n, out, valid, T);
    return hipGetLastError();
}

#define PLAN_THREADS 256
#define PLAN_NV 7
enum { PV_SYM = 0, PV_BYTE, PV_DW, PV_OUT, PV_MF, PV_JOB, PV_VB };

__device__ __forceinline__ unsigned pll_class(unsigned ms)
{
    switch (ms) {
    case FX_MODEM_PSK2: return 0; case FX_MODEM_PSK4: return 1; case FX_MODEM_PSK8: return 2; case FX_MODEM_PSK16: return 3;
    case FX_MODEM_DPSK2: return 4; case FX_MODEM_DPSK4: return 5; case FX_MODEM_DPSK8: return 6; case FX_MODEM_ASK4: return 7;
    case FX_MODEM_QAM16: return 8; case FX_MODEM_QAM32: return 9; case FX_MODEM_QAM64: return 10; default: return 11;
    }
}

__device__ __forceinline__ void plan_scan(uint32_t (&v)[PLAN_NV], uint32_t (&tot)[PLAN_NV], uint32_t (*ws)[PLAN_NV])
{
    const int tid = threadIdx.x, lane = tid & 63, wave = tid >> 6;
    uint32_t inc[PLAN_NV];
#pragma unroll
    for (int q = 0; q < PLAN_NV; q++) {
        inc[q] = v[q];
#pragma unroll
        for (int d = 1; d < 64; d <<= 1) { const uint32_t o = (uint32_t)__shfl_up((int)inc[q], d, 64); if (lane >= d) inc[q] += o; }
    }
    __syncthreads();
    if (lane == 63) for (int q = 0; q < PLAN_NV; q++) ws[wave][q] = inc[q];
    __syncthreads();
#pragma unroll
    for (int q = 0; q < PLAN_NV; q++) {
        uint32_t wb = 0, t = 0;
#pragma unroll
        for (int w = 0; w < PLAN_THREADS / 64; w++) { const uint32_t x = ws[w][q]; if (w < wave) wb += x; t += x; }
        tot[q] = t; v[q] = wb + inc[q] - v[q];
    }
}

#define PLAN_MAXG 256
enum { PW_TICKET = 0, PW_CLS_CNT = 16, PW_DEC_CNT = 28, PW_VBC_CNT = 31, PW_CLS_FILL = 38, PW_DEC_FILL = 50, PW_VBC_FILL = 53,
       PW_FLAG = 128, PW_AGG = 384, PW_INC = 384 + 8 * PLAN_MAXG, PW_WORDS = 384 + 16 * PLAN_MAXG };

__device__ __forceinline__ uint32_t wave_agg_add(uint32_t *counters, uint32_t key, uint32_t inc, bool active)
{
    const int lane = threadIdx.x & 63;
    unsigned long long rem = __ballot(active);
    uint32_t result = 0;
    while (rem) {
        const int leader = __ffsll((long long)rem) - 1;
        const uint32_t k = (uint32_t)__shfl((int)key, leader, 64);
        const bool mine = active && key == k;
        const unsigned long long same = __ballot(mine);
        uint32_t incl = mine ? inc : 0u;
#pragma unroll
        for (int d = 1; d < 64; d <<= 1) { const uint32_t o = (uint32_t)__shfl_up((int)incl, d, 64); if (lane >= d) incl += o; }
        const uint32_t total = (uint32_t)__shfl((int)incl, 63, 64);
        uint32_t base = 0;
        if (lane == leader) base = atomicAdd(&counters[k], total);
        base = (uint32_t)__shfl((int)base, leader, 64);
        if (mine) result = base + incl - inc;
        rem &= ~same;
    }
    return result;
}

struct PlanWords { uint32_t flags, nsym, plen, ms, check, fec0, fec1; };
__device__ __forceinline__ PlanWords plan_words(const FxFrame *fp) { return { fp->flags, fp->pay_sym_len, fp->pay_len, fp->ms, fp->check, fp->fec0, fp->fec1 }; }
struct PlanFrame {
    const FxFrame *fp = nullptr; uint32_t sidx = 0, bps = 0, k = 0, l0 = 0, l1 = 0, nblk = 0, vnb = 0; bool valid = false, batch = false;
};
__device__ __forceinline__ PlanFrame plan_sizes(const PlanWords &w, bool live, uint32_t detect, uint32_t vb_blk, uint32_t (&v)[PLAN_NV])
{
    PlanFrame f;
#pragma unroll
    for (int q = 0; q < PLAN_NV; q++) v[q] = 0u;
    f.valid = live && !detect && (w.flags & FX_FLAG_HEADER_VALID);
    if (!f.valid) return f;
    f.bps = modem_bps(w.ms);
    f.k = w.plen + crc_len(w.check); f.l0 = fec_enc_len(w.fec0, f.k); f.l1 = fec_enc_len(w.fec1, f.l0);
    f.nblk = (w.nsym + 1023u) / 1024u;
    v[PV_SYM] = (w.nsym + 7u) & ~7u;
    v[PV_BYTE] = (max(f.l1, f.k) + 8u + 15u) & ~15u;
    v[PV_DW] = ((8u * max(f.l0, f.k) + 6u + 63u) & ~63u) + 64u;
    v[PV_OUT] = (w.plen + 15u) & ~15u;
    v[PV_MF] = f.nblk; v[PV_JOB] = 1u;
    f.batch = vb_blk && conv_p(w.fec0) && !conv_p(w.fec1) && w.fec1 != FX_FEC_RS_M8;
    if (f.batch) { f.vnb = (8u * f.k + 6u + vb_blk - 1u) / vb_blk; v[PV_VB] = f.vnb; }
    return f;
}
__device__ __forceinline__ bool plan_demote(uint32_t vb_before, uint32_t vnb, uint32_t vb_cap) { return (uint64_t)vb_before + vnb + 7u * 128u > vb_cap; }

struct PlanKey {
    uint32_t cls, rs, vc;
    __device__ uint32_t dec(bool batch) const { return batch ? 2u : rs; }
    __device__ uint32_t pack() const { return cls | rs << 4 | vc << 5; }
    __device__ static PlanKey unpack(uint32_t p) { return { p & 15u, (p >> 4) & 1u, (p >> 5) & 7u }; }
};
__device__ __forceinline__ PlanKey plan_key(uint32_t ms, uint32_t fec0, uint32_t fec1)
{
    const uint32_t p = (uint32_t)conv_p(fec0);
    return { pll_class(ms), (fec0 == FX_FEC_RS_M8 || fec1 == FX_FEC_RS_M8) ? 1u : 0u, p ? p - 1u : 0u };
}

__device__ __forceinline__ uint32_t plan_stream_of(const uint32_t *base, uint32_t nstreams, uint32_t g)
{
    uint32_t lo = 0, hi = nstreams;
    while (hi - lo > 1) { const uint32_t mid = (lo + hi) >> 1; if (base[mid] <= g) lo = mid; else hi = mid; }
    return lo;
}

__device__ __forceinline__ void plan_emit(FxPayJob *__restrict__ job, FxOutRec *__restrict__ rec, const FxFrame *__restrict__ fp, const FxStreamDesc *__restrict__ sd,
                                          const PlanWords &w, const PlanFrame &f, const uint32_t (&off)[PLAN_NV], uint32_t eq, uint32_t slot, uint32_t vb_off)
{
    FxPayJob j;
    j.x = sd->x; j.xa_end = sd->xa_end; j.start = fp->start; j.mix_th = fp->mix_th; j.mix_dl = fp->mix_dl; j.mf_scale = fp->mf_scale;
    j.pfb = fp->pfb; j.mfc0 = fp->mfc0; j.pll_th = fp->pll_th; j.pll_f = fp->pll_f; j.ms = w.ms; j.bps = f.bps;
    j.nsym = f.valid ? w.nsym : 0u; j.sym_off = off[PV_SYM];
    j.pay_len = w.plen; j.check = w.check; j.fec0 = w.fec0; j.fec1 = w.fec1; j.k = f.k; j.l0 = f.l0; j.l1 = f.l1;
    j.byte_off = off[PV_BYTE]; j.dw_off = off[PV_DW]; j.out_off = off[PV_OUT]; j.pad_ = f.valid ? 1u : 0u;
    j.eq = eq; j.chain_idx = slot; j.vb_off = vb_off; j.vb_nblk = (uint16_t)f.vnb; j.vb_clean = 0;
    *job = j;
    union { FxOutRec r; uint4 q[sizeof(FxOutRec) / 16]; } u;
    u.r.start = sd->abs_base + fp->start; u.r.stream = f.sidx; u.r.offset = fp->offset;
    u.r.rxy = fp->rxy; u.r.tau = fp->tau; u.r.gamma = fp->gamma; u.r.dphi = fp->dphi; u.r.phi = fp->phi; u.r.pfb = fp->pfb;
    u.r.pilot_dphi = fp->pilot_dphi; u.r.pilot_phi = fp->pilot_phi; u.r.pilot_gain = fp->pilot_gain;
    u.r.flags = w.flags & FX_FLAG_HEADER_VALID;
    u.r.pay_len = f.valid ? w.plen : 0u; u.r.ms = w.ms; u.r.check = w.check; u.r.fec0 = w.fec0; u.r.fec1 = w.fec1;
    u.r.nsym = f.valid ? w.nsym : 0u; u.r.bps = f.bps; u.r.sym_off = off[PV_SYM]; u.r.out_off = off[PV_OUT];
    u.r.evm_sum = 0.0f; u.r.payload_valid = 0; u.r.status = 0;
    const uint32_t *hw = reinterpret_cast<const uint32_t *>(fp->header); uint32_t *rw = reinterpret_cast<uint32_t *>(u.r.header);
#pragma unroll
    for (int i = 0; i < FX_HDR_DEC / 4; i++) rw[i] = hw[i];
    u.r.byte_off = off[PV_BYTE];
    uint4 *dst = reinterpret_cast<uint4 *>(rec);
#pragma unroll
    for (int i = 0; i < (int)(sizeof(FxOutRec) / 16); i++) dst[i] = u.q[i];
}

template <bool AGENT> struct PlanCounts {
    const uint32_t *cls_, *dec_, *vbc_;
    __device__ __forceinline__ static uint32_t ld(const uint32_t *p)
    {
        if constexpr (AGENT) return __hip_atomic_load(p, __ATOMIC_RELAXED, __HIP_MEMORY_SCOPE_AGENT); else return *p;
    }
    __device__ __forceinline__ uint32_t cls(int c) const { return ld(cls_ + c); }
    __device__ __forceinline__ uint32_t dec(int c) const { return ld(dec_ + c); }
    __device__ __forceinline__ uint32_t vbc(int c) const { return ld(vbc_ + c); }
};
template <class Counts> __device__ __forceinline__ void plan_class_bases(const Counts &cnt, uint32_t (&cls_base)[FX_PLL_CLASSES + 1], uint32_t (&vbc_base)[8])
{
    uint32_t b = 0;
    for (int c = 0; c < FX_PLL_CLASSES; c++) { cls_base[c] = b; b += (cnt.cls(c) + 63u) & ~63u; }
    cls_base[FX_PLL_CLASSES] = b;
    uint32_t vb = 0;
    for (int c = 0; c < 7; c++) { vbc_base[c] = vb; vb += (cnt.vbc(c) + 127u) & ~127u; }
    vbc_base[7] = vb;
}
template <class Counts> __device__ __forceinline__ void plan_pad_lists(const Counts &cnt, const uint32_t (&cls_base)[FX_PLL_CLASSES + 1], const uint32_t (&vbc_base)[8], const FxPlanArgs &a)
{
    for (int c = 0; c < FX_PLL_CLASSES; c++)
        for (uint32_t i = cls_base[c] + cnt.cls(c) + threadIdx.x; i < cls_base[c + 1] && i < a.list_cap; i += PLAN_THREADS) a.pll_list[i] = 0xFFFFFFFFu;
    for (int c = 0; c < 7; c++)
        for (uint32_t i = vbc_base[c] + cnt.vbc(c) + threadIdx.x; i < vbc_base[c + 1] && i < a.vb_cap; i += PLAN_THREADS) a.vb_items[i] = 0xFFFFFFFFu;
}
template <class Tot, class Counts> __device__ __forceinline__ void plan_fill_hdr(FxBlockHdr &h, uint32_t N, Tot tot, const Counts &cnt, const uint32_t (&cls_base)[FX_PLL_CLASSES + 1],
                                                                                 const uint32_t (&vbc_base)[8], const FxPlanArgs &a)
{
    h.n_frames = N; h.n_pjobs = tot[PV_JOB]; h.n_mfblk = min(tot[PV_MF], a.mf_cap);
    h.n_dec_plain = cnt.dec(0); h.n_dec_rs = cnt.dec(1); h.n_dec_batch = cnt.dec(2);
    h.n_vb_items = min(vbc_base[7], a.vb_cap); h.vb_blk = a.vb_blk; h.vb_want = tot[PV_VB] + 7u * 128u; h.n_vb_fallback = 0;
    for (int c = 0; c < FX_PLL_CLASSES; c++) { h.pll_cnt[c] = cnt.cls(c); h.pll_base[c] = cls_base[c]; }
    h.pll_base[FX_PLL_CLASSES] = cls_base[FX_PLL_CLASSES];
    h.sym_total = tot[PV_SYM]; h.byte_total = tot[PV_BYTE]; h.dw_total = tot[PV_DW]; h.out_total = tot[PV_OUT];
    h.done = 1;
}
__device__ __forceinline__ void plan_mirror_hdr(const FxBlockHdr &h, const FxPlanArgs &a)
{
    const uint32_t *src = reinterpret_cast<const uint32_t *>(&h);
    uint32_t *d0 = reinterpret_cast<uint32_t *>(a.hdr_pay), *d1 = reinterpret_cast<uint32_t *>(a.hdr_host), *z = reinterpret_cast<uint32_t *>(a.hdr);
    for (int i = threadIdx.x; i < (int)(sizeof(FxBlockHdr) / 4); i += PLAN_THREADS) { const uint32_t w = src[i]; d0[i] = w; d1[i] = w; z[i] = 0u; }
}

__device__ __forceinline__ PlanFrame plan_frame(uint32_t g, bool live, const FxPlanArgs &a, PlanWords &w, uint32_t (&v)[PLAN_NV])
{
    const uint32_t sidx = live ? plan_stream_of(a.stream_base, a.nstreams, g) : 0u;
    const FxFrame *fp = live ? a.chain + a.streams[sidx].chain_base + (g - a.stream_base[sidx]) : nullptr;
    w = live ? plan_words(fp) : PlanWords{};
    PlanFrame f = plan_sizes(w, live, a.detect, a.vb_blk, v);
    f.fp = fp; f.sidx = sidx;
    return f;
}
__device__ __forceinline__ void plan_range(uint32_t N, uint32_t &g0, uint32_t &g1)
{
    const uint32_t per = ((N + gridDim.x - 1) / gridDim.x + PLAN_THREADS - 1) / PLAN_THREADS * PLAN_THREADS;
    g0 = min(N, blockIdx.x * per); g1 = min(N, g0 + per);
}
__device__ __forceinline__ uint32_t plan_stream_bases(const uint32_t *chain_count, uint32_t nstreams, uint32_t *stream_base, uint32_t (*ws)[PLAN_NV])
{
    const int tid = threadIdx.x;
    uint32_t run = 0;
    for (uint32_t s0 = 0; s0 < nstreams; s0 += PLAN_THREADS) {
        const uint32_t sidx = s0 + tid;
        uint32_t v[PLAN_NV] = { sidx < nstreams ? chain_count[sidx] : 0u, 0, 0, 0, 0, 0, 0 }, tot[PLAN_NV];
        plan_scan(v, tot, ws);
        if (sidx < nstreams) stream_base[sidx] = run + v[0];
        run += tot[0];
        __syncthreads();
    }
    if (tid == 0) stream_base[nstreams] = run;
    __threadfence(); __syncthreads(); __threadfence();
    return run;
}

extern "C" __global__ __launch_bounds__(PLAN_THREADS)
void fx_plan_kernel(const FxPlanArgs a)
{
    __shared__ uint32_t ws[PLAN_THREADS / 64][PLAN_NV];
    __shared__ uint32_t base_s[PLAN_NV];
    uint32_t *const pw = a.ws;
    const int tid = threadIdx.x;
    const uint32_t N = plan_stream_bases(a.chain_count, a.nstreams, a.stream_base, ws);
    uint32_t g0, g1; plan_range(N, g0, g1);
    const uint32_t wg = blockIdx.x;
    uint32_t run[PLAN_NV] = { 0, 0, 0, 0, 0, 0, 0 };
    for (uint32_t c0 = g0; c0 < g1; c0 += PLAN_THREADS) {
        uint32_t v[PLAN_NV], tot[PLAN_NV]; PlanWords w;
        (void)plan_frame(c0 + tid, c0 + tid < g1, a, w, v);
        plan_scan(v, tot, ws);
#pragma unroll
        for (int q = 0; q < PLAN_NV; q++) run[q] += tot[q];
        __syncthreads();
    }
    if (tid == 0) {
        uint32_t base[PLAN_NV] = { 0, 0, 0, 0, 0, 0, 0 };
        if (wg > 0) {
            for (int q = 0; q < PLAN_NV; q++) pw[PW_AGG + 8 * wg + q] = run[q];
            __threadfence();
            __hip_atomic_store(&pw[PW_FLAG + wg], 1u, __ATOMIC_RELEASE, __HIP_MEMORY_SCOPE_AGENT);
            for (int p = (int)wg - 1; p >= 0; p--) {
                uint32_t f;
                do { f = __hip_atomic_load(&pw[PW_FLAG + p], __ATOMIC_ACQUIRE, __HIP_MEMORY_SCOPE_AGENT); if (!f) __builtin_amdgcn_s_sleep(2); } while (!f);
                const volatile uint32_t *src = pw + (f == 2u ? PW_INC : PW_AGG) + 8 * p;
                for (int q = 0; q < PLAN_NV; q++) base[q] += src[q];
                if (f == 2u) break;
            }
        }
        for (int q = 0; q < PLAN_NV; q++) { pw[PW_INC + 8 * wg + q] = base[q] + run[q]; base_s[q] = base[q]; }
        __threadfence();
        __hip_atomic_store(&pw[PW_FLAG + wg], 2u, __ATOMIC_RELEASE, __HIP_MEMORY_SCOPE_AGENT);
    }
    __syncthreads();
    uint32_t before[PLAN_NV];
#pragma unroll
    for (int q = 0; q < PLAN_NV; q++) before[q] = base_s[q];
    for (uint32_t c0 = g0; c0 < g1; c0 += PLAN_THREADS) {
        const uint32_t g = c0 + tid;
        const bool live = g < g1;
        uint32_t v[PLAN_NV], tot[PLAN_NV]; PlanWords w;
        PlanFrame f = plan_frame(g, live, a, w, v);
        plan_scan(v, tot, ws);
#pragma unroll
        for (int q = 0; q < PLAN_NV; q++) { v[q] += before[q]; before[q] += tot[q]; }
        if (f.batch && plan_demote(v[PV_VB], f.vnb, a.vb_cap)) { f.batch = false; f.vnb = 0; }
        if (live) {
            plan_emit(a.pjobs + g, a.recs + g, f.fp, a.streams + f.sidx, w, f, v, a.eq, (uint32_t)(f.fp - a.chain), 0u);
            for (uint32_t c = 0; c < f.nblk; c++) if (v[PV_MF] + c < a.mf_cap) { a.mf_job[v[PV_MF] + c] = g; a.mf_c0[v[PV_MF] + c] = c * 1024u; }
        }
        {
            const PlanKey key = plan_key(w.ms, w.fec0, w.fec1);
            (void)wave_agg_add(pw + PW_CLS_CNT, key.cls, 1u, f.valid);
            (void)wave_agg_add(pw + PW_DEC_CNT, key.dec(f.batch), 1u, f.valid);
            (void)wave_agg_add(pw + PW_VBC_CNT, key.vc, f.vnb, f.batch);
        }
        __syncthreads();
    }
}

extern "C" __global__ __launch_bounds__(PLAN_THREADS)
void fx_planlists_kernel(const FxPlanArgs a)
{
    __shared__ struct { FxBlockHdr h; uint32_t cls_base[FX_PLL_CLASSES + 1], vbc_base[8], last; } sh;
    uint32_t *const pw = a.ws;
    const PlanCounts<true> cnt{ pw + PW_CLS_CNT, pw + PW_DEC_CNT, pw + PW_VBC_CNT };
    const int tid = threadIdx.x;
    const uint32_t N = __hip_atomic_load(&a.stream_base[a.nstreams], __ATOMIC_RELAXED, __HIP_MEMORY_SCOPE_AGENT);
    if (tid == 0) plan_class_bases(cnt, sh.cls_base, sh.vbc_base);
    __syncthreads();
    uint32_t g0, g1; plan_range(N, g0, g1);
    for (uint32_t c0 = g0; c0 < g1; c0 += PLAN_THREADS) {
        const uint32_t g = c0 + tid;
        const bool live = g < g1;
        uint32_t ms = 0, fec0 = 0, fec1 = 0, vnb = 0; bool val = false;
        if (live) { const FxPayJob &j = a.pjobs[g]; val = j.pad_ != 0; ms = j.ms; fec0 = j.fec0; fec1 = j.fec1; vnb = j.vb_nblk; }
        const PlanKey key = plan_key(ms, fec0, fec1);
        const bool bt = val && vnb;
        const uint32_t pp = sh.cls_base[key.cls] + wave_agg_add(pw + PW_CLS_FILL, key.cls, 1u, val);
        if (val && pp < a.list_cap) a.pll_list[pp] = g;
        const uint32_t rs = key.dec(bt), dp = wave_agg_add(pw + PW_DEC_FILL, rs, 1u, val);
        if (val && dp < a.list_cap) a.dec_list[(size_t)rs * a.list_cap + dp] = g;
        const uint32_t at = sh.vbc_base[key.vc] + wave_agg_add(pw + PW_VBC_FILL, key.vc, vnb, bt);
        if (bt) {
            for (uint32_t b = 0; b < vnb; b++) if (at + b < a.vb_cap) { a.vb_items[at + b] = g; a.vb_items[a.vb_cap + at + b] = b; }
            a.pjobs[g].vb_off = at;
        }
    }
    if (blockIdx.x == 0) plan_pad_lists(cnt, sh.cls_base, sh.vbc_base, a);
    __threadfence(); __syncthreads();
    if (tid == 0) sh.last = atomicAdd(&pw[PW_TICKET], 1u) == gridDim.x - 1 ? 1u : 0u;
    __syncthreads();
    if (!sh.last) return;
    __threadfence();
    if (tid == 0) {
        sh.h = *a.hdr;
        plan_fill_hdr(sh.h, N, (const volatile uint32_t *)(pw + PW_INC + 8 * (gridDim.x - 1)), cnt, sh.cls_base, sh.vbc_base, a);
    }
    __syncthreads();
    plan_mirror_hdr(sh.h, a);
    for (int i = tid; i < PW_WORDS; i += PLAN_THREADS) pw[i] = 0u;
}

#define PLAN_KEEP 8
#define PLAN_LDS_STREAMS 256
enum { PO_CLS = 0, PO_DEC = FX_PLL_CLASSES, PO_VBC = FX_PLL_CLASSES + 4, PO_N = FX_PLL_CLASSES + 12 };
struct PlanOneShared {
    FxBlockHdr h;
    uint32_t ws[PLAN_THREADS / 64][PLAN_NV];
    uint32_t cnt[PO_N], fill[PO_N];
    uint32_t cls_base[FX_PLL_CLASSES + 1], vbc_base[8];
    uint32_t sbase[PLAN_LDS_STREAMS + 1], cbase[PLAN_LDS_STREAMS];
};
__device__ __forceinline__ uint32_t plan_one_slot(uint32_t g, const FxPlanArgs &a, const PlanOneShared &sh, uint32_t &sidx)
{
    if (a.nstreams <= PLAN_LDS_STREAMS) { sidx = plan_stream_of(sh.sbase, a.nstreams, g); return sh.cbase[sidx] + (g - sh.sbase[sidx]); }
    sidx = plan_stream_of(a.stream_base, a.nstreams, g);
    return a.streams[sidx].chain_base + (g - a.stream_base[sidx]);
}

extern "C" __global__ __launch_bounds__(PLAN_THREADS)
void fx_planfused_kernel(const FxPlanArgs a)
{
    __shared__ PlanOneShared sh;
    __shared__ uint4 keep[PLAN_KEEP * PLAN_THREADS];
    constexpr uint32_t TILE = PLAN_KEEP * PLAN_THREADS;
    const PlanCounts<false> cnt{ sh.cnt + PO_CLS, sh.cnt + PO_DEC, sh.cnt + PO_VBC };
    const uint32_t tid = threadIdx.x, nstreams = a.nstreams;
#ifdef FX_STAMPS
    unsigned long long tk_ = __builtin_readcyclecounter(); uint32_t st1_ = 0, st2_ = 0, st6_ = 0, st7_ = 0;
#define PLAN_TICK(acc) do { const unsigned long long t_ = __builtin_readcyclecounter(); acc += (uint32_t)(t_ - tk_); tk_ = t_; } while (0)
#else
#define PLAN_TICK(acc) do { } while (0)
#endif
    {
        const uint32_t *src = reinterpret_cast<const uint32_t *>(a.hdr); uint32_t *dst = reinterpret_cast<uint32_t *>(&sh.h);
        for (int i = (int)tid; i < (int)(sizeof(FxBlockHdr) / 4); i += PLAN_THREADS) dst[i] = src[i];
        if (tid < PO_N) { sh.cnt[tid] = 0u; sh.fill[tid] = 0u; }
        if (tid <= FX_PLL_CLASSES) sh.cls_base[tid] = 0u;
        if (tid < 8) sh.vbc_base[tid] = 0u;
    }
    uint32_t N;
    if (nstreams <= PLAN_LDS_STREAMS) {
        uint32_t v[PLAN_NV] = { tid < nstreams ? a.chain_count[tid] : 0u, 0, 0, 0, 0, 0, 0 }, tot[PLAN_NV];
        if (nstreams > 1) plan_scan(v, tot, sh.ws); else { tot[0] = v[0]; v[0] = 0u; }
        if (tid < nstreams) { sh.sbase[tid] = v[0]; a.stream_base[tid] = v[0]; sh.cbase[tid] = a.streams[tid].chain_base; }
        if (tid == 0) { sh.sbase[nstreams] = tot[0]; a.stream_base[nstreams] = tot[0]; }
        __syncthreads();
        N = sh.sbase[nstreams];
    } else N = plan_stream_bases(a.chain_count, nstreams, a.stream_base, sh.ws);

    uint32_t run[PLAN_NV] = { 0, 0, 0, 0, 0, 0, 0 };
    for (int pass = N > TILE ? 0 : 1; pass < 2; pass++) {
#pragma unroll
        for (int q = 0; q < PLAN_NV; q++) run[q] = 0u;
        for (uint32_t t0 = 0; t0 < N; t0 += TILE) {
            const uint32_t nt = min(TILE, N - t0), t1 = t0 + nt, per = (nt + PLAN_THREADS - 1) / PLAN_THREADS, f0 = t0 + tid * per;
            uint32_t st[PLAN_NV], tot[PLAN_NV];
            uint32_t info[PLAN_KEEP];
            {
                PlanWords w[PLAN_KEEP];
#pragma unroll
                for (int i = 0; i < PLAN_KEEP; i++) {
                    const bool live = (uint32_t)i < per && f0 + i < t1;
                    uint32_t sidx;
                    w[i] = plan_words(a.chain + plan_one_slot(live ? f0 + i : t0, a, sh, sidx));
                }
#pragma unroll
                for (int q = 0; q < PLAN_NV; q++) st[q] = 0u;
#pragma unroll
                for (int i = 0; i < PLAN_KEEP; i++) {
                    uint32_t v[PLAN_NV];
                    const PlanFrame f = plan_sizes(w[i], (uint32_t)i < per && f0 + i < t1, a.detect, a.vb_blk, v);
                    info[i] = f.valid ? f.vnb | plan_key(w[i].ms, w[i].fec0, w[i].fec1).pack() << 16 | 1u << 24 | (f.batch ? 1u << 25 : 0u) : 0u;
#pragma unroll
                    for (int q = 0; q < PLAN_NV; q++) st[q] += v[q];
                }
            }
            plan_scan(st, tot, sh.ws);
#pragma unroll
            for (int q = 0; q < PLAN_NV; q++) st[q] += run[q];
            if (pass == 0 || N <= TILE) {
                uint32_t vb = st[PV_VB];
#pragma unroll
                for (int i = 0; i < PLAN_KEEP; i++) {
                    const uint32_t vnb = info[i] & 0xffffu;
                    const bool batch = ((info[i] >> 25) & 1u) && !plan_demote(vb, vnb, a.vb_cap);
                    vb += vnb;
                    if ((info[i] >> 24) & 1u) {
                        const PlanKey key = PlanKey::unpack(info[i] >> 16);
                        atomicAdd(&sh.cnt[PO_CLS + key.cls], 1u);
                        atomicAdd(&sh.cnt[PO_DEC + key.dec(batch)], 1u);
                        if (batch) atomicAdd(&sh.cnt[PO_VBC + key.vc], vnb);
                    }
                }
            }
            if (pass == 0) {
#pragma unroll
                for (int q = 0; q < PLAN_NV; q++) run[q] += tot[q];
                continue;
            }
            if (t0 == 0) {
                __syncthreads();
                if (tid == 0) plan_class_bases(cnt, sh.cls_base, sh.vbc_base);
                __syncthreads();
            }
            PLAN_TICK(st1_);
            for (uint32_t i = 0; i < per && f0 + i < t1; i++) {
                const uint32_t g = f0 + i;
                uint32_t sidx, v[PLAN_NV];
                const uint32_t slot = plan_one_slot(g, a, sh, sidx);
                const FxFrame *fp = a.chain + slot;
                const PlanWords w = plan_words(fp);
                PlanFrame f = plan_sizes(w, true, a.detect, a.vb_blk, v);
                f.fp = fp; f.sidx = sidx;
                if (f.batch && plan_demote(st[PV_VB], f.vnb, a.vb_cap)) { f.batch = false; f.vnb = 0; }
                uint32_t at = 0;
                if (f.valid) {
                    const PlanKey key = plan_key(w.ms, w.fec0, w.fec1);
                    const uint32_t pp = sh.cls_base[key.cls] + atomicAdd(&sh.fill[PO_CLS + key.cls], 1u);
                    if (pp < a.list_cap) a.pll_list[pp] = g;
                    const uint32_t rs = key.dec(f.batch), dp = atomicAdd(&sh.fill[PO_DEC + rs], 1u);
                    if (dp < a.list_cap) a.dec_list[(size_t)rs * a.list_cap + dp] = g;
                    if (f.batch) at = sh.vbc_base[key.vc] + atomicAdd(&sh.fill[PO_VBC + key.vc], f.vnb);
                }
                keep[g - t0] = make_uint4(at, f.vnb, st[PV_MF], f.nblk);
                plan_emit(a.pjobs + g, a.recs + g, fp, a.streams + sidx, w, f, st, a.eq, slot, at);
#pragma unroll
                for (int q = 0; q < PLAN_NV; q++) st[q] += v[q];
            }
            __syncthreads();
            PLAN_TICK(st2_);
            for (uint32_t k = tid >> 4; k < nt; k += PLAN_THREADS / 16) {
                const uint4 kp = keep[k];
                const uint32_t g = t0 + k, sub = tid & 15u;
                for (uint32_t b = sub; b < kp.y; b += 16u) if (kp.x + b < a.vb_cap) { a.vb_items[kp.x + b] = g; a.vb_items[a.vb_cap + kp.x + b] = b; }
                for (uint32_t c = sub; c < kp.w; c += 16u) if (kp.z + c < a.mf_cap) { a.mf_job[kp.z + c] = g; a.mf_c0[kp.z + c] = c * 1024u; }
            }
#pragma unroll
            for (int q = 0; q < PLAN_NV; q++) run[q] += tot[q];
            __syncthreads();
        }
    }
    plan_pad_lists(cnt, sh.cls_base, sh.vbc_base, a);
    PLAN_TICK(st6_);
    __threadfence(); __syncthreads();
    PLAN_TICK(st7_);
    if (tid == 0) {
#ifdef FX_STAMPS
        sh.h.stamp[1] = st1_; sh.h.stamp[2] = st2_; sh.h.stamp[6] = st6_; sh.h.stamp[7] = st7_;
#endif
        plan_fill_hdr(sh.h, N, run, cnt, sh.cls_base, sh.vbc_base, a);
    }
    __syncthreads();
    plan_mirror_hdr(sh.h, a);
}

extern "C" hipError_t fx_launch_plan(hipStream_t st, unsigned grid, int fused, const FxPlanArgs &a)
{
    const unsigned g = grid < 1u ? 1u : (grid > PLAN_MAXG ? PLAN_MAXG : grid);
    if (fused && g == 1u) hipLaunchKernelGGL(fx_planfused_kernel, dim3(1), dim3(PLAN_THREADS), 0, st, a);
    else {
        hipLaunchKernelGGL(fx_plan_kernel, dim3(g), dim3(PLAN_THREADS), 0, st, a);
        hipLaunchKernelGGL(fx_planlists_kernel, dim3(g), dim3(PLAN_THREADS), 0, st, a);
    }
    return hipGetLastError();
}
extern "C" unsigned fx_plan_ws_words(void) { return PW_WORDS; }

#define PMF_THREADS 256
#define PMF_SYMS    1024
#define PMF_SPAN    (2 * PMF_SYMS + FX_MF_TAPS)

template <bool EQ>
__global__ __launch_bounds__(PMF_THREADS)
void fx_paymf_kernel(const FxPayJob *jobs, const uint32_t *blk_job, const uint32_t *blk_c0, const FxBlockHdr *hdr, const FxFrame *chain, float2 *sym_raw,
                     const FxTables *T)
{
    constexpr int LEAD = EQ ? FX_EQ_TAPS - 1 : 0;
    __shared__ float2 v[PMF_SPAN + LEAD + 4];
    __shared__ float2 u[EQ ? 2 * PMF_SYMS + FX_EQ_TAPS : 1];
    __shared__ float2 eqw[16];
    __shared__ float taps[FX_MF_TAPS];
    const uint32_t nitems = hdr->n_mfblk;
    const int tid = threadIdx.x;
    const float2 *sc = T->sc;
    for (uint32_t bi = blockIdx.x; bi < nitems; bi += gridDim.x) {
        const FxPayJob job = jobs[blk_job[bi]];
        const uint32_t c0 = blk_c0[bi];
        const uint32_t ns = min((uint32_t)PMF_SYMS, job.nsym - c0);
        const int64_t sym0 = (int64_t)FX_SYM0_PAY + (EQ ? FX_EQ_DELAY : 0);
        const int64_t nlo = sym_sample(sym0 + c0, job.mfc0) - LEAD - (FX_MF_TAPS - 1);
        const int64_t nhi = sym_sample(sym0 + c0 + ns - 1, job.mfc0);
        const int span = (int)(nhi - nlo + 1);
        const XSrc xs = make_xsrc(job.x, job.xa_end, 0);
        __syncthreads();
        if (tid < FX_MF_TAPS) taps[tid] = T->proto[job.pfb + FX_NPFB * tid];
        if (EQ && tid < 16) eqw[tid] = tid < FX_EQ_TAPS ? chain[job.chain_idx].eq[tid] : make_float2(0.0f, 0.0f);
        for (int m = tid; m < span; m += PMF_THREADS) {
            const int64_t nn = nlo + m;
            v[m] = derot(xld(xs, job.start + nn), job.mix_th + job.mix_dl * (uint32_t)nn, sc);
        }
        __syncthreads();
        if (EQ) {
            const int nu = span - (FX_MF_TAPS - 1);
            for (int m = tid; m < nu; m += PMF_THREADS) {
                float ar = 0.0f, ai = 0.0f;
#pragma unroll 7
                for (int t = 0; t < FX_MF_TAPS; t++) {
                    const float2 w = v[m + (FX_MF_TAPS - 1) - t]; const float h = taps[t];
                    ar = fmaf(h, w.x, ar); ai = fmaf(h, w.y, ai);
                }
                u[m] = make_float2(ar * job.mf_scale, ai * job.mf_scale);
            }
            __syncthreads();
            for (uint32_t i = tid; i < ns; i += PMF_THREADS) {
                const int nc = (int)(sym_sample(sym0 + c0 + i, job.mfc0) - nlo) - (FX_MF_TAPS - 1);
                sym_raw[(size_t)job.sym_off + c0 + i] = eq_sum16(u + nc - (FX_EQ_TAPS - 1), eqw);
            }
        } else {
            for (uint32_t i = tid; i < ns; i += PMF_THREADS) {
                const int nc = (int)(sym_sample(sym0 + c0 + i, job.mfc0) - nlo);
                float ar = 0.0f, ai = 0.0f;
#pragma unroll 7
                for (int t = 0; t < FX_MF_TAPS; t++) {
                    const float2 w = v[nc - t]; const float h = taps[t];
                    ar = fmaf(h, w.x, ar); ai = fmaf(h, w.y, ai);
                }
                sym_raw[(size_t)job.sym_off + c0 + i] = make_float2(ar * job.mf_scale, ai * job.mf_scale);
            }
        }
    }
}

#define PMF4_STRIDE 274
extern "C" __global__ __launch_bounds__(PMF_THREADS)
void fx_paymf4_kernel(const FxPayJob *jobs, const uint32_t *blk_job, const uint32_t *blk_c0, const FxBlockHdr *hdr, float2 *sym_raw, const FxTables *T)
{
    __shared__ float2 ph[8 * PMF4_STRIDE];
    __shared__ __attribute__((aligned(16))) float taps[FX_MF_TAPS];
    static_assert(FX_MF_TAPS == 28 && PMF_SYMS == 4 * PMF_THREADS, "tile below: 28 taps, four symbols per thread");
    static_assert(PMF4_STRIDE >= (PMF_SPAN + 8) / 8 + 5, "phase arrays hold the span plus the slack phantom symbols read");
    const uint32_t nitems = hdr->n_mfblk;
    const int tid = threadIdx.x;
    const float2 *sc = T->sc;
    for (uint32_t bi = blockIdx.x; bi < nitems; bi += gridDim.x) {
        const FxPayJob job = jobs[blk_job[bi]];
        const uint32_t c0 = blk_c0[bi];
        const uint32_t ns = min((uint32_t)PMF_SYMS, job.nsym - c0);
        const int64_t nlo = sym_sample((int64_t)FX_SYM0_PAY + c0, job.mfc0) - (FX_MF_TAPS - 1);
        const int span = 2 * (int)ns + (FX_MF_TAPS - 2);
        const float2 *px = job.x, *pa = job.xa_end;
        const int64_t p0 = job.start + nlo;
        const uint32_t th0 = job.mix_th + job.mix_dl * (uint32_t)nlo, dl = job.mix_dl;
        __syncthreads();
        if (tid < FX_MF_TAPS) taps[tid] = T->proto[job.pfb + FX_NPFB * tid];
        constexpr int NLD = (PMF_SPAN + PMF_THREADS - 1) / PMF_THREADS;
        float2 raw[NLD];
#pragma unroll
        for (int k = 0; k < NLD; k++) {
            const int m = tid + PMF_THREADS * k;
            const int64_t p = p0 + m;
            raw[k] = m < span ? (p < 0 ? pa[p] : px[p]) : make_float2(0.0f, 0.0f);
        }
#pragma unroll
        for (int k = 0; k < NLD; k++) {
            const int m = tid + PMF_THREADS * k;
            const int j = m >> 1;
            if (m < span) ph[((m & 1) * 4 + (j & 3)) * PMF4_STRIDE + (j >> 2)] = derot(raw[k], th0 + dl * (uint32_t)m, sc);
        }
        __syncthreads();
        if (4u * (uint32_t)tid < ns) {
            float2 e[17], o[17];
#pragma unroll
            for (int j = 0; j < 17; j++) {
                e[j] = ph[(j & 3) * PMF4_STRIDE + tid + (j >> 2)];
                o[j] = ph[(4 + (j & 3)) * PMF4_STRIDE + tid + (j >> 2)];
            }
            float h[FX_MF_TAPS];
#pragma unroll
            for (int q = 0; q < FX_MF_TAPS / 4; q++) { const float4 t4 = reinterpret_cast<const float4 *>(taps)[q]; h[4 * q] = t4.x; h[4 * q + 1] = t4.y; h[4 * q + 2] = t4.z; h[4 * q + 3] = t4.w; }
            float yr[4], yi[4];
#pragma unroll
            for (int r = 0; r < 4; r++) {
                float ar = 0.0f, ai = 0.0f;
#pragma unroll
                for (int k = 0; k < 14; k++) {
                    ar = fmaf(h[2 * k], o[13 + r - k].x, ar); ai = fmaf(h[2 * k], o[13 + r - k].y, ai);
                    ar = fmaf(h[2 * k + 1], e[13 + r - k].x, ar); ai = fmaf(h[2 * k + 1], e[13 + r - k].y, ai);
                }
                yr[r] = ar * job.mf_scale; yi[r] = ai * job.mf_scale;
            }
            float4 *dst = reinterpret_cast<float4 *>(sym_raw + (size_t)job.sym_off + c0 + 4u * (uint32_t)tid);
            dst[0] = make_float4(yr[0], yi[0], yr[1], yi[1]);
            dst[1] = make_float4(yr[2], yi[2], yr[3], yi[3]);
        }
    }
}

extern "C" hipError_t fx_launch_paymf(unsigned grid, int eq, hipStream_t st, const FxPayJob *jobs, const uint32_t *blk_job, const uint32_t *blk_c0, const FxBlockHdr *hdr,
                                      const FxFrame *chain, float2 *sym_raw, const FxTables *T)
{
    if (grid == 0) return hipSuccess;
    if (eq) hipLaunchKernelGGL(fx_paymf_kernel<true>, dim3(grid), dim3(PMF_THREADS), 0, st, jobs, blk_job, blk_c0, hdr, chain, sym_raw, T);
    else hipLaunchKernelGGL(fx_paymf4_kernel, dim3(grid), dim3(PMF_THREADS), 0, st, jobs, blk_job, blk_c0, hdr, sym_raw, T);
    return hipGetLastError();
}

#define PLL_THREADS 64
#define PLL_MAX_WAVES 4
#define PLL_BLK     8

__device__ __forceinline__ void pll_load8(const float4 *p, float4 b[4]) { b[0] = p[0]; b[1] = p[1]; b[2] = p[2]; b[3] = p[3]; }

template <int MS>
__device__ __forceinline__ unsigned pll_demod(float2 r, unsigned &prev, const float2 *sc, float2 &xh, float &pe)
{
    if constexpr (MS == FX_MODEM_PSK2 || MS == FX_MODEM_PSK4) {
        unsigned idx; float pr, pim;
        if constexpr (MS == FX_MODEM_PSK2) {
            const bool neg = !(r.x > 0.0f);
            idx = neg ? 1u : 0u;
            xh = make_float2(neg ? -1.0f : 1.0f, 0.0f);
            pr = neg ? -r.x : r.x; pim = neg ? -r.y : r.y;
        } else {
            const bool horiz = fabsf(r.x) >= fabsf(r.y);
            const bool neg = horiz ? !(r.x > 0.0f) : !(r.y > 0.0f);
            idx = (horiz ? 0u : 1u) + (neg ? 2u : 0u);
            const float sg = neg ? -1.0f : 1.0f;
            xh = horiz ? make_float2(sg, 0.0f) : make_float2(0.0f, sg);
            const float a = horiz ? r.x : r.y, b = horiz ? r.y : -r.x;
            pr = neg ? -a : a; pim = neg ? -b : b;
        }
        (void)pr;
        pe = pim;
        return gray_enc(idx);
    } else {
        return modem_demod((unsigned)MS, modem_bps((unsigned)MS), r, prev, sc, xh, pe);
    }
}

template <int MS, bool TAIL>
__device__ __forceinline__ void pll_block8(const float4 (&cur)[4], unsigned live, uint32_t &th, float &fq, float &evm, unsigned &prev, const float2 *sc,
                                           float4 *out, uint2 *hd)
{
    float rr[2 * PLL_BLK]; unsigned h0 = 0, h1 = 0;
    float wc, ws; sincos_u32(th, sc, wc, ws);
#pragma unroll
    for (int k = 0; k < PLL_BLK; k++) {
        const float4 v4 = cur[k >> 1];
        const float2 y = (k & 1) ? make_float2(v4.z, v4.w) : make_float2(v4.x, v4.y);
        float2 r = make_float2(fmaf(y.x, wc, y.y * ws), fmaf(y.y, wc, -(y.x * ws))), xh; float pe;
        unsigned pv = prev;
        const unsigned s = pll_demod<MS>(r, pv, sc, xh, pe);
        if (!TAIL || (unsigned)k < live) {
            float dr = r.x - xh.x, di = r.y - xh.y;
            evm += fmaf(dr, dr, di * di);
            fq = fmaf(pe, 68356.5248f, fq);
            const float t = phase_step(fmaf(pe, 6835652.5f, fq));
            th += (uint32_t)(int)t;
            float cd, sd; sincos_small(t, cd, sd);
            const float c2 = fmaf(wc, cd, -(ws * sd)), s2 = fmaf(ws, cd, wc * sd);
            wc = c2; ws = s2;
            prev = pv;
        }
        rr[2 * k] = r.x; rr[2 * k + 1] = r.y;
        if (k < 4) h0 |= s << (8 * k); else h1 |= s << (8 * (k - 4));
    }
#pragma unroll
    for (int k = 0; k < 4; k++) out[k] = make_float4(rr[4 * k], rr[4 * k + 1], rr[4 * k + 2], rr[4 * k + 3]);
    *hd = make_uint2(h0, h1);
}

template <int MS>
__device__ __forceinline__ void pll_frame(uint32_t f, const FxPayJob *jobs, const float2 *sc, const float2 *sym_raw, float2 *framesyms, uint8_t *hard, FxOutRec *recs)
{
    if (f == 0xFFFFFFFFu) return;
    const FxPayJob job = jobs[f];
    const float4 *in = reinterpret_cast<const float4 *>(sym_raw + job.sym_off);
    float4 *out = reinterpret_cast<float4 *>(framesyms + job.sym_off);
    uint2 *hd = reinterpret_cast<uint2 *>(hard + job.sym_off);
    uint32_t th = job.pll_th; float fq = job.pll_f * 683565248.0f, evm = 0.0f; unsigned prev = 0;
    const unsigned nsym = job.nsym;
    const uint32_t nfull = nsym / PLL_BLK, rem = nsym % PLL_BLK;
    float4 cur[4], nxt[4];
    if (nsym) pll_load8(in, cur);
    for (uint32_t b = 0; b < nfull; b++) {
        if ((b + 1) * PLL_BLK < nsym) pll_load8(in + 4 * (b + 1), nxt);
        pll_block8<MS, false>(cur, PLL_BLK, th, fq, evm, prev, sc, out + 4 * b, hd + b);
#pragma unroll
        for (int k = 0; k < 4; k++) cur[k] = nxt[k];
    }
    if (rem) pll_block8<MS, true>(cur, rem, th, fq, evm, prev, sc, out + 4 * nfull, hd + nfull);
    recs[f].evm_sum = evm;
}

__global__ __launch_bounds__(PLL_THREADS * PLL_MAX_WAVES)
void fx_paypll_kernel(const FxPllGang g, const FxTables *T)
{
    const FxPllMember m = g.m[blockIdx.y];
    const FxBlockHdr *hdr = m.hdr;
    const uint32_t nw = hdr->pll_base[FX_PLL_CLASSES] >> 6;
    const uint32_t wpg = blockDim.x >> 6, w0 = blockIdx.x * wpg + (threadIdx.x >> 6);
    if (blockIdx.x * wpg >= nw) return;
    __builtin_amdgcn_s_setprio(3);
    __shared__ float2 sc[1024];
    for (int i = threadIdx.x; i < 1024; i += blockDim.x) sc[i] = T->sc[i];
    __syncthreads();
    const int lane = threadIdx.x & 63;
    for (uint32_t w = w0; w < nw; w += gridDim.x * wpg) {
        uint32_t cls = 0;
        while (cls + 1 < FX_PLL_CLASSES && (w << 6) >= hdr->pll_base[cls + 1]) cls++;
        cls = __builtin_amdgcn_readfirstlane(cls);
        const uint32_t f = m.pll_list[(w << 6) + lane];
#define FX_PLL_CASE(C, M) case C: pll_frame<M>(f, m.jobs, sc, m.sym_raw, m.framesyms, m.hard, m.recs); break;
        switch (cls) {
            FX_PLL_CASE(0, FX_MODEM_PSK2) FX_PLL_CASE(1, FX_MODEM_PSK4) FX_PLL_CASE(2, FX_MODEM_PSK8) FX_PLL_CASE(3, FX_MODEM_PSK16)
            FX_PLL_CASE(4, FX_MODEM_DPSK2) FX_PLL_CASE(5, FX_MODEM_DPSK4) FX_PLL_CASE(6, FX_MODEM_DPSK8) FX_PLL_CASE(7, FX_MODEM_ASK4)
            FX_PLL_CASE(8, FX_MODEM_QAM16) FX_PLL_CASE(9, FX_MODEM_QAM32) FX_PLL_CASE(10, FX_MODEM_QAM64)
            default: pll_frame<FX_MODEM_QPSK>(f, m.jobs, sc, m.sym_raw, m.framesyms, m.hard, m.recs); break;
        }
#undef FX_PLL_CASE
    }
}

extern "C" hipError_t fx_launch_paypll(const FxPllGang *gang, const unsigned *grid_waves, unsigned waves_per_wg, hipStream_t st, const FxTables *T)
{
    if (gang->n > FX_GANG_MAX) return hipErrorInvalidValue;
    FxPllGang g; g.n = 0;
    unsigned gw = 0;
    for (uint32_t i = 0; i < gang->n; i++) if (grid_waves[i]) { g.m[g.n++] = gang->m[i]; gw = grid_waves[i] > gw ? grid_waves[i] : gw; }
    if (g.n == 0) return hipSuccess;
    for (uint32_t i = g.n; i < FX_GANG_MAX; i++) g.m[i] = g.m[0];
    const unsigned w = waves_per_wg < 1u ? 1u : (waves_per_wg > PLL_MAX_WAVES ? PLL_MAX_WAVES : waves_per_wg);
    hipLaunchKernelGGL(fx_paypll_kernel, dim3((gw + w - 1) / w, g.n), dim3(PLL_THREADS * w), 0, st, g, T);
    return hipGetLastError();
}

#define DEC_THREADS 64

__device__ __forceinline__ unsigned getbit(const uint8_t *b, uint32_t i) { return (b[i >> 3] >> (7 - (i & 7))) & 1u; }

__device__ __forceinline__ void permute_bits(const uint8_t *src, uint8_t *dst, const uint32_t *perm, uint32_t nbytes, int lane)
{
    for (uint32_t j = lane; j < nbytes; j += DEC_THREADS) {
        unsigned v = 0;
#pragma unroll
        for (int b = 0; b < 8; b++) v = (v << 1) | getbit(src, perm[8 * j + b]);
        dst[j] = (uint8_t)v;
    }
}

__device__ __forceinline__ void deinterleave_wave(uint8_t *x, uint32_t n, int lane)
{
    if (n < 2) return;
    const uint32_t M = 1u + (uint32_t)floorf(sqrtf((float)n));
    uint32_t N = n / M; while (n >= M * N) N++;
    const uint32_t n2 = n / 2, nn0 = n / 3, step_q = 64u / M, step_m = 64u % M;
    for (int p = 3; p >= 0; p--) {
        const uint32_t Np = N + (p == 0 ? 0u : (p == 1 ? 2u : (p == 2 ? 4u : 8u)));
        const uint32_t mk = p == 0 ? 0xffu : (p == 1 ? 0x0fu : (p == 2 ? 0x55u : 0x33u));
        uint32_t m = (uint32_t)lane % M, q = (uint32_t)lane / M, i_base = 0;
        const uint32_t max_iter = (M * (Np + 1u)) / 64u + 2u;
        for (uint32_t it = 0; i_base < n2 && it < max_iter; it++) {
            const uint32_t nn = q == 0 ? nn0 : (nn0 + q) % Np;
// ... 2098 lines not shown
```

gr-liquiddsp_amd/csrc/fx_launch.h:

```cpp
#pragma once
#include <hip/hip_runtime.h>
#include "fx_common.h"

struct FxTables;

extern "C" hipError_t fx_launch_walk(unsigned mode, int eq, int sh, unsigned njobs, hipStream_t st, const FxWalkJob *jobs, const uint32_t *job_list, FxWalkResult *results,
                                     FxFrame *frames, FxVerifyRun *runs, uint32_t run_cap, FxBlockHdr *hdr, const FxTables *T, int ext, uint32_t n_jobs_total,
                                     const uint32_t *n_list, uint32_t list_cap);
extern "C" hipError_t fx_launch_prescan(hipStream_t st, unsigned n_spec, unsigned words_per_job, const FxWalkJob *jobs, const uint32_t *spec_list, const FxTables *T);
extern "C" hipError_t fx_launch_seekverify(unsigned grid, hipStream_t st, const FxVerifyRun *runs, uint32_t run_cap, const FxWalkJob *jobs, FxWalkResult *results,
                                           FxFrame *frames, FxBlockHdr *hdr, const FxTables *T, uint32_t phase);
extern "C" hipError_t fx_launch_chain(unsigned mode, int eq, int sh, unsigned nstreams, hipStream_t st, const FxStreamDesc *streams, const FxWalkJob *jobs, uint32_t n_jobs_total,
                                      FxWalkResult *results, FxFrame *frames, FxFrame *chain, uint32_t *chain_count, FxVerifyRun *runs, uint32_t run_cap,
                                      FxBlockHdr *hdr, uint32_t force_slow, const FxTables *T);
extern "C" hipError_t fx_launch_hdrdec(int soft, unsigned n, hipStream_t st, const uint8_t *in, uint8_t *out, int32_t *valid, const FxTables *T);
extern "C" hipError_t fx_launch_blkdec(int soft, unsigned fs, unsigned n, unsigned count, hipStream_t st, const uint8_t *in, uint8_t *out, const FxTables *T);
extern "C" hipError_t fx_launch_blksiso(unsigned fs, unsigned n, unsigned count, hipStream_t st, const uint8_t *in, uint8_t *out, const FxTables *T);
extern "C" hipError_t fx_launch_rssoft(unsigned n, unsigned count, hipStream_t st, const uint8_t *in, uint8_t *out, uint8_t *chosen_f, const FxTables *T);
extern "C" hipError_t fx_launch_chainfast(unsigned nstreams, hipStream_t st, const FxStreamDesc *streams, const FxWalkJob *jobs, const FxWalkResult *results,
                                          const FxFrame *frames, FxFrame *chain, uint32_t *chain_count, FxBlockHdr *hdr, uint32_t force_repair,
                                          FxWalkJob *jobs_rw, uint32_t *req_list, uint32_t *stat, uint32_t pass);
extern "C" hipError_t fx_launch_plan(hipStream_t st, unsigned grid, int fused, const FxPlanArgs &a);
extern "C" unsigned fx_plan_ws_words(void);
extern "C" hipError_t fx_launch_vbpre(const FxVbpreGang *gang, hipStream_t st, const FxTables *T, int clean_on, int early_tail);
extern "C" hipError_t fx_launch_vbitems(unsigned first_item, unsigned n_items, hipStream_t st, const FxPayJob *jobs, const uint32_t *vb_items, uint32_t item_cap,
                                        const FxBlockHdr *hdr, uint8_t *bufA, const uint8_t *bufB, unsigned long long *dwv, uint8_t *vec_arena, uint32_t *vb_st, uint32_t dbg, int packed,
                                        int with_fix);
extern "C" hipError_t fx_launch_vbfinish(unsigned first_wave, unsigned n_waves, hipStream_t st, const FxPayJob *jobs, const uint32_t *job_idx, FxBlockHdr *hdr,
                                         uint8_t *bufA, uint8_t *bufB, unsigned long long *dwv, const uint8_t *vec_arena, const uint32_t *vb_st, uint32_t *fb_list, uint32_t list_cap,
                                         uint8_t *out, FxOutRec *recs, FxBlockHdr *hdr_host, int early_tail);
extern "C" hipError_t fx_launch_paymf(unsigned grid, int eq, hipStream_t st, const FxPayJob *jobs, const uint32_t *blk_job, const uint32_t *blk_c0, const FxBlockHdr *hdr,
                                      const FxFrame *chain, float2 *sym_raw, const FxTables *T);
extern "C" hipError_t fx_launch_paypll(const FxPllGang *gang, const unsigned *grid_waves, unsigned waves_per_wg, hipStream_t st, const FxTables *T);
extern "C" hipError_t fx_launch_paydec(int with_rs, int soft, int soft_rs, unsigned first_wave, unsigned grid_waves, unsigned waves_per_wg, hipStream_t st, const FxPayJob *jobs,
                                       const uint32_t *job_idx, const FxBlockHdr *hdr, const uint8_t *hard, uint8_t *bufA, uint8_t *bufB, uint8_t *soft_arena,
                                       unsigned long long *dw_arena, uint8_t *out, FxOutRec *recs, FxPayResult *res, const FxTables *T, FxBlockHdr *fallback_host);
extern "C" hipError_t fx_launch_symcopy(unsigned grid, hipStream_t st, const FxBlockHdr *hdr, const float2 *sym, float2 *host);
extern "C" hipError_t fx_launch_upload(hipStream_t st, const void *src, void *dst, size_t bytes, unsigned n_cus);
extern "C" hipError_t fx_launch_ingest(hipStream_t st, int fmt, const void *src, float2 *dst, size_t n, float scale, unsigned n_cus);
extern "C" hipError_t fx_launch_detwin(hipStream_t st, unsigned grid, const FxStreamDesc *streams, uint32_t nstreams, const uint32_t *stream_base, const FxPayJob *pjobs,
                                       const FxBlockHdr *hdr, uint32_t first, uint32_t reserved, float2 *out, float2 *out_tail, uint32_t *flag_host, int with_tails,
                                       int skip_tail);
extern "C" hipError_t fx_launch_copy_u32(hipStream_t st, const uint32_t *src, uint32_t *dst);
extern "C" hipError_t fx_launch_softdemod(unsigned grid, hipStream_t st, const FxPayJob *jobs, const uint32_t *blk_job, const uint32_t *blk_c0, const FxBlockHdr *hdr,
                                          const float2 *framesyms, const uint8_t *hard, uint8_t *soft_arena, const FxTables *T);

extern "C" hipError_t fx_launch_txgen(unsigned ntiles, hipStream_t st, const FxTxJob *jobs, const uint32_t *tile_job, const uint32_t *tile_n0,
                                      const uint8_t *head_idx, const uint8_t *pay_idx, const FxTxTables *T, float2 *out);
extern "C" hipError_t fx_launch_txenc(unsigned njobs, hipStream_t st, const FxTxEncJob *jobs, const uint8_t *pay, const uint32_t *perm_arena,
                                      uint8_t *bufA, uint8_t *bufB, uint8_t *pay_idx, const FxTxTables *T);
extern "C" hipError_t fx_launch_channel(hipStream_t st, float2 *x, unsigned n_streams, unsigned long long n_per_stream, const FxChannel *chs, const FxTxTables *T);
extern "C" hipError_t fx_launch_quantize(hipStream_t st, int fmt, const float2 *in, void *out, size_t n, float inv_scale, unsigned long long *saturated,
                                         unsigned n_cus);
```

Measured before the change: 37940 Msamples/s.

## Template fused plan kernel on thread count and preload frame words per tile

The single-block fused planning kernel is templated on block size (256 or 512, selectable by environment, default 512) with a fixed 2048-frame tile. Each thread now loads its frames' header words and slots up front into registers and reuses them in both the counting and emit phases, instead of packing info bits and reloading them later. Emit also batches loads of the remaining frame and stream fields two at a time so global loads overlap. The cost is higher register pressure per thread from the KEEP-sized arrays of PlanWords.

```diff
diff --git a/gr-liquiddsp_amd/csrc/fx_host.cpp b/gr-liquiddsp_amd/csrc/fx_host.cpp
--- a/gr-liquiddsp_amd/csrc/fx_host.cpp
+++ b/gr-liquiddsp_amd/csrc/fx_host.cpp
@@ -173,6 +173,7 @@
     bool vb_clean = true;
     int inchain_repair = 1; unsigned inchain_left = 0;
     bool plan_fused = true;
+    unsigned plan_threads = 512;
     bool vb_early_tail = true;
     int timing_level = -1;
     hipEvent_t ref_event = nullptr; double ref_host_ms = 0.0;
@@ -395,6 +396,7 @@
     if (const char *e = std::getenv("FXRX_VB_CLEAN")) c->vb_clean = std::atoi(e) != 0;
     if (const char *e = std::getenv("FXRX_INCHAIN_REPAIR")) c->inchain_repair = std::min(2, std::max(0, std::atoi(e)));
     if (const char *e = std::getenv("FXRX_PLAN_FUSED")) c->plan_fused = std::atoi(e) != 0;
+    if (const char *e = std::getenv("FXRX_PLAN_THREADS")) { const int v = std::atoi(e); if (v == 256 || v == 512) c->plan_threads = (unsigned)v; }
     if (const char *e = std::getenv("FXRX_VB_EARLY_TAIL")) c->vb_early_tail = std::atoi(e) != 0;
     if (const char *e = std::getenv("FXRX_DEBUG_STOP_AFTER")) c->debug_stop_after = std::atoi(e);
     if (const char *e = std::getenv("FXRX_DEBUG_WALK_TWICE")) c->debug_walk_twice = std::atoi(e);
@@ -806,7 +808,7 @@
         a.pll_list = sl.d_pll_list.p; a.dec_list = sl.dec_list(kDecPlain); a.list_cap = sl.list_cap();
         a.vb_items = sl.d_vb_items.p; a.vb_cap = sl.vb_cap;
         a.hdr = sl.hdr_walk(); a.hdr_pay = sl.hdr_pay(); a.hdr_host = sl.h_hdr.p; a.ws = sl.d_plan_ws.p;
-        HIP_OK(fx_launch_plan(st, c->plan_grid ? c->plan_grid : (unsigned)std::min<uint64_t>(64, c->traffic.frames / 2048 + 1), c->plan_fused ? 1 : 0, a));
+        HIP_OK(fx_launch_plan(st, c->plan_grid ? c->plan_grid : (unsigned)std::min<uint64_t>(64, c->traffic.frames / 2048 + 1), c->plan_fused ? 1 : 0, c->plan_threads, a));
     }
     const int tl = sl.timing_level;
     if (tl >= 2) HIP_OK(hipEventRecord(sl.ev[kEvPlan], st));
diff --git a/gr-liquiddsp_amd/csrc/fx_kernels.hip b/gr-liquiddsp_amd/csrc/fx_kernels.hip
--- a/gr-liquiddsp_amd/csrc/fx_kernels.hip
+++ b/gr-liquiddsp_amd/csrc/fx_kernels.hip
@@ -1694,7 +1694,7 @@
     }
 }
 
-__device__ __forceinline__ void plan_scan(uint32_t (&v)[PLAN_NV], uint32_t (&tot)[PLAN_NV], uint32_t (*ws)[PLAN_NV])
+template <int NT> __device__ __forceinline__ void plan_scan(uint32_t (&v)[PLAN_NV], uint32_t (&tot)[PLAN_NV], uint32_t (*ws)[PLAN_NV])
 {
     const int tid = threadIdx.x, lane = tid & 63, wave = tid >> 6;
     uint32_t inc[PLAN_NV];
@@ -1711,7 +1711,7 @@
     for (int q = 0; q < PLAN_NV; q++) {
         uint32_t wb = 0, t = 0;
 #pragma unroll
-        for (int w = 0; w < PLAN_THREADS / 64; w++) { const uint32_t x = ws[w][q]; if (w < wave) wb += x; t += x; }
+        for (int w = 0; w < NT / 64; w++) { const uint32_t x = ws[w][q]; if (w < wave) wb += x; t += x; }
         tot[q] = t; v[q] = wb + inc[q] - v[q];
     }
 }
@@ -1788,28 +1788,45 @@
     return lo;
 }
 
-__device__ __forceinline__ void plan_emit(FxPayJob *__restrict__ job, FxOutRec *__restrict__ rec, const FxFrame *__restrict__ fp, const FxStreamDesc *__restrict__ sd,
+struct PlanRest {
+    const float2 *x, *xa_end; int64_t abs_base;
+    int64_t start; int32_t offset; float rxy, tau, gamma, dphi, phi; uint32_t pfb; int32_t mfc0; uint32_t mix_th, mix_dl; float mf_scale;
+    float pilot_dphi, pilot_phi, pilot_gain; uint32_t pll_th; float pll_f; uint32_t header[FX_HDR_DEC / 4];
+};
+__device__ __forceinline__ PlanRest plan_rest(const FxFrame *__restrict__ fp, const FxStreamDesc *__restrict__ sd)
+{
+    PlanRest r;
+    r.x = sd->x; r.xa_end = sd->xa_end; r.abs_base = sd->abs_base;
+    r.start = fp->start; r.offset = fp->offset; r.rxy = fp->rxy; r.tau = fp->tau; r.gamma = fp->gamma; r.dphi = fp->dphi; r.phi = fp->phi;
+    r.pfb = fp->pfb; r.mfc0 = fp->mfc0; r.mix_th = fp->mix_th; r.mix_dl = fp->mix_dl; r.mf_scale = fp->mf_scale;
+    r.pilot_dphi = fp->pilot_dphi; r.pilot_phi = fp->pilot_phi; r.pilot_gain = fp->pilot_gain; r.pll_th = fp->pll_th; r.pll_f = fp->pll_f;
+    const uint32_t *hw = reinterpret_cast<const uint32_t *>(fp->header);
+#pragma unroll
+    for (int i = 0; i < FX_HDR_DEC / 4; i++) r.header[i] = hw[i];
+    return r;
+}
+__device__ __forceinline__ void plan_emit(FxPayJob *__restrict__ job, FxOutRec *__restrict__ rec, const PlanRest &fp,
                                           const PlanWords &w, const PlanFrame &f, const uint32_t (&off)[PLAN_NV], uint32_t eq, uint32_t slot, uint32_t vb_off)
 {
     FxPayJob j;
-    j.x = sd->x; j.xa_end = sd->xa_end; j.start = fp->start; j.mix_th = fp->mix_th; j.mix_dl = fp->mix_dl; j.mf_scale = fp->mf_scale;
-    j.pfb = fp->pfb; j.mfc0 = fp->mfc0; j.pll_th = fp->pll_th; j.pll_f = fp->pll_f; j.ms = w.ms; j.bps = f.bps;
+    j.x = fp.x; j.xa_end = fp.xa_end; j.start = fp.start; j.mix_th = fp.mix_th; j.mix_dl = fp.mix_dl; j.mf_scale = fp.mf_scale;
+    j.pfb = fp.pfb; j.mfc0 = fp.mfc0; j.pll_th = fp.pll_th; j.pll_f = fp.pll_f; j.ms = w.ms; j.bps = f.bps;
     j.nsym = f.valid ? w.nsym : 0u; j.sym_off = off[PV_SYM];
     j.pay_len = w.plen; j.check = w.check; j.fec0 = w.fec0; j.fec1 = w.fec1; j.k = f.k; j.l0 = f.l0; j.l1 = f.l1;
     j.byte_off = off[PV_BYTE]; j.dw_off = off[PV_DW]; j.out_off = off[PV_OUT]; j.pad_ = f.valid ? 1u : 0u;
     j.eq = eq; j.chain_idx = slot; j.vb_off = vb_off; j.vb_nblk = (uint16_t)f.vnb; j.vb_clean = 0;
     *job = j;
     union { FxOutRec r; uint4 q[sizeof(FxOutRec) / 16]; } u;
-    u.r.start = sd->abs_base + fp->start; u.r.stream = f.sidx; u.r.offset = fp->offset;
-    u.r.rxy = fp->rxy; u.r.tau = fp->tau; u.r.gamma = fp->gamma; u.r.dphi = fp->dphi; u.r.phi = fp->phi; u.r.pfb = fp->pfb;
-    u.r.pilot_dphi = fp->pilot_dphi; u.r.pilot_phi = fp->pilot_phi; u.r.pilot_gain = fp->pilot_gain;
+    u.r.start = fp.abs_base + fp.start; u.r.stream = f.sidx; u.r.offset = fp.offset;
+    u.r.rxy = fp.rxy; u.r.tau = fp.tau; u.r.gamma = fp.gamma; u.r.dphi = fp.dphi; u.r.phi = fp.phi; u.r.pfb = fp.pfb;
+    u.r.pilot_dphi = fp.pilot_dphi; u.r.pilot_phi = fp.pilot_phi; u.r.pilot_gain = fp.pilot_gain;
     u.r.flags = w.flags & FX_FLAG_HEADER_VALID;
     u.r.pay_len = f.valid ? w.plen : 0u; u.r.ms = w.ms; u.r.check = w.check; u.r.fec0 = w.fec0; u.r.fec1 = w.fec1;
     u.r.nsym = f.valid ? w.nsym : 0u; u.r.bps = f.bps; u.r.sym_off = off[PV_SYM]; u.r.out_off = off[PV_OUT];
     u.r.evm_sum = 0.0f; u.r.payload_valid = 0; u.r.status = 0;
-    const uint32_t *hw = reinterpret_cast<const uint32_t *>(fp->header); uint32_t *rw = reinterpret_cast<uint32_t *>(u.r.header);
-#pragma unroll
-    for (int i = 0; i < FX_HDR_DEC / 4; i++) rw[i] = hw[i];
+    uint32_t *rw = reinterpret_cast<uint32_t *>(u.r.header);
+#pragma unroll
+    for (int i = 0; i < FX_HDR_DEC / 4; i++) rw[i] = fp.header[i];
     u.r.byte_off = off[PV_BYTE];
     uint4 *dst = reinterpret_cast<uint4 *>(rec);
 #pragma unroll
@@ -1835,12 +1852,12 @@
     for (int c = 0; c < 7; c++) { vbc_base[c] = vb; vb += (cnt.vbc(c) + 127u) & ~127u; }
     vbc_base[7] = vb;
 }
-template <class Counts> __device__ __forceinline__ void plan_pad_lists(const Counts &cnt, const uint32_t (&cls_base)[FX_PLL_CLASSES + 1], const uint32_t (&vbc_base)[8], const FxPlanArgs &a)
+template <int NT, class Counts> __device__ __forceinline__ void plan_pad_lists(const Counts &cnt, const uint32_t (&cls_base)[FX_PLL_CLASSES + 1], const uint32_t (&vbc_base)[8], const FxPlanArgs &a)
 {
     for (int c = 0; c < FX_PLL_CLASSES; c++)
-        for (uint32_t i = cls_base[c] + cnt.cls(c) + threadIdx.x; i < cls_base[c + 1] && i < a.list_cap; i += PLAN_THREADS) a.pll_list[i] = 0xFFFFFFFFu;
+        for (uint32_t i = cls_base[c] + cnt.cls(c) + threadIdx.x; i < cls_base[c + 1] && i < a.list_cap; i += NT) a.pll_list[i] = 0xFFFFFFFFu;
     for (int c = 0; c < 7; c++)
-        for (uint32_t i = vbc_base[c] + cnt.vbc(c) + threadIdx.x; i < vbc_base[c + 1] && i < a.vb_cap; i += PLAN_THREADS) a.vb_items[i] = 0xFFFFFFFFu;
+        for (uint32_t i = vbc_base[c] + cnt.vbc(c) + threadIdx.x; i < vbc_base[c + 1] && i < a.vb_cap; i += NT) a.vb_items[i] = 0xFFFFFFFFu;
 }
 template <class Tot, class Counts> __device__ __forceinline__ void plan_fill_hdr(FxBlockHdr &h, uint32_t N, Tot tot, const Counts &cnt, const uint32_t (&cls_base)[FX_PLL_CLASSES + 1],
                                                                                  const uint32_t (&vbc_base)[8], const FxPlanArgs &a)
@@ -1853,11 +1870,11 @@
     h.sym_total = tot[PV_SYM]; h.byte_total = tot[PV_BYTE]; h.dw_total = tot[PV_DW]; h.out_total = tot[PV_OUT];
     h.done = 1;
 }
-__device__ __forceinline__ void plan_mirror_hdr(const FxBlockHdr &h, const FxPlanArgs &a)
+template <int NT> __device__ __forceinline__ void plan_mirror_hdr(const FxBlockHdr &h, const FxPlanArgs &a)
 {
     const uint32_t *src = reinterpret_cast<const uint32_t *>(&h);
     uint32_t *d0 = reinterpret_cast<uint32_t *>(a.hdr_pay), *d1 = reinterpret_cast<uint32_t *>(a.hdr_host), *z = reinterpret_cast<uint32_t *>(a.hdr);
-    for (int i = threadIdx.x; i < (int)(sizeof(FxBlockHdr) / 4); i += PLAN_THREADS) { const uint32_t w = src[i]; d0[i] = w; d1[i] = w; z[i] = 0u; }
+    for (int i = threadIdx.x; i < (int)(sizeof(FxBlockHdr) / 4); i += NT) { const uint32_t w = src[i]; d0[i] = w; d1[i] = w; z[i] = 0u; }
 }
 
 __device__ __forceinline__ PlanFrame plan_frame(uint32_t g, bool live, const FxPlanArgs &a, PlanWords &w, uint32_t (&v)[PLAN_NV])
@@ -1874,14 +1891,14 @@
     const uint32_t per = ((N + gridDim.x - 1) / gridDim.x + PLAN_THREADS - 1) / PLAN_THREADS * PLAN_THREADS;
     g0 = min(N, blockIdx.x * per); g1 = min(N, g0 + per);
 }
-__device__ __forceinline__ uint32_t plan_stream_bases(const uint32_t *chain_count, uint32_t nstreams, uint32_t *stream_base, uint32_t (*ws)[PLAN_NV])
+template <int NT> __device__ __forceinline__ uint32_t plan_stream_bases(const uint32_t *chain_count, uint32_t nstreams, uint32_t *stream_base, uint32_t (*ws)[PLAN_NV])
 {
     const int tid = threadIdx.x;
     uint32_t run = 0;
-    for (uint32_t s0 = 0; s0 < nstreams; s0 += PLAN_THREADS) {
+    for (uint32_t s0 = 0; s0 < nstreams; s0 += NT) {
         const uint32_t sidx = s0 + tid;
         uint32_t v[PLAN_NV] = { sidx < nstreams ? chain_count[sidx] : 0u, 0, 0, 0, 0, 0, 0 }, tot[PLAN_NV];
-        plan_scan(v, tot, ws);
+        plan_scan<NT>(v, tot, ws);
         if (sidx < nstreams) stream_base[sidx] = run + v[0];
         run += tot[0];
         __syncthreads();
@@ -1898,14 +1915,14 @@
     __shared__ uint32_t base_s[PLAN_NV];
     uint32_t *const pw = a.ws;
     const int tid = threadIdx.x;
-    const uint32_t N = plan_stream_bases(a.chain_count, a.nstreams, a.stream_base, ws);
+    const uint32_t N = plan_stream_bases<PLAN_THREADS>(a.chain_count, a.nstreams, a.stream_base, ws);
     uint32_t g0, g1; plan_range(N, g0, g1);
     const uint32_t wg = blockIdx.x;
     uint32_t run[PLAN_NV] = { 0, 0, 0, 0, 0, 0, 0 };
     for (uint32_t c0 = g0; c0 < g1; c0 += PLAN_THREADS) {
         uint32_t v[PLAN_NV], tot[PLAN_NV]; PlanWords w;
         (void)plan_frame(c0 + tid, c0 + tid < g1, a, w, v);
-        plan_scan(v, tot, ws);
+        plan_scan<PLAN_THREADS>(v, tot, ws);
 #pragma unroll
         for (int q = 0; q < PLAN_NV; q++) run[q] += tot[q];
         __syncthreads();
@@ -1937,12 +1954,12 @@
         const bool live = g < g1;
         uint32_t v[PLAN_NV], tot[PLAN_NV]; PlanWords w;
         PlanFrame f = plan_frame(g, live, a, w, v);
-        plan_scan(v, tot, ws);
+        plan_scan<PLAN_THREADS>(v, tot, ws);
 #pragma unroll
         for (int q = 0; q < PLAN_NV; q++) { v[q] += before[q]; before[q] += tot[q]; }
         if (f.batch && plan_demote(v[PV_VB], f.vnb, a.vb_cap)) { f.batch = false; f.vnb = 0; }
         if (live) {
-            plan_emit(a.pjobs + g, a.recs + g, f.fp, a.streams + f.sidx, w, f, v, a.eq, (uint32_t)(f.fp - a.chain), 0u);
+            plan_emit(a.pjobs + g, a.recs + g, plan_rest(f.fp, a.streams + f.sidx), w, f, v, a.eq, (uint32_t)(f.fp - a.chain), 0u);
             for (uint32_t c = 0; c < f.nblk; c++) if (v[PV_MF] + c < a.mf_cap) { a.mf_job[v[PV_MF] + c] = g; a.mf_c0[v[PV_MF] + c] = c * 1024u; }
         }
         {
@@ -1983,7 +2000,7 @@
             a.pjobs[g].vb_off = at;
         }
     }
-    if (blockIdx.x == 0) plan_pad_lists(cnt, sh.cls_base, sh.vbc_base, a);
+    if (blockIdx.x == 0) plan_pad_lists<PLAN_THREADS>(cnt, sh.cls_base, sh.vbc_base, a);
     __threadfence(); __syncthreads();
     if (tid == 0) sh.last = atomicAdd(&pw[PW_TICKET], 1u) == gridDim.x - 1 ? 1u : 0u;
     __syncthreads();
@@ -1994,33 +2011,36 @@
         plan_fill_hdr(sh.h, N, (const volatile uint32_t *)(pw + PW_INC + 8 * (gridDim.x - 1)), cnt, sh.cls_base, sh.vbc_base, a);
     }
     __syncthreads();
-    plan_mirror_hdr(sh.h, a);
+    plan_mirror_hdr<PLAN_THREADS>(sh.h, a);
     for (int i = tid; i < PW_WORDS; i += PLAN_THREADS) pw[i] = 0u;
 }
 
-#define PLAN_KEEP 8
+#define PLAN_TILE 2048
+#define PLAN_BATCH 2
 #define PLAN_LDS_STREAMS 256
 enum { PO_CLS = 0, PO_DEC = FX_PLL_CLASSES, PO_VBC = FX_PLL_CLASSES + 4, PO_N = FX_PLL_CLASSES + 12 };
-struct PlanOneShared {
+template <int NT> struct PlanOneShared {
     FxBlockHdr h;
-    uint32_t ws[PLAN_THREADS / 64][PLAN_NV];
+    uint32_t ws[NT / 64][PLAN_NV];
     uint32_t cnt[PO_N], fill[PO_N];
     uint32_t cls_base[FX_PLL_CLASSES + 1], vbc_base[8];
     uint32_t sbase[PLAN_LDS_STREAMS + 1], cbase[PLAN_LDS_STREAMS];
 };
-__device__ __forceinline__ uint32_t plan_one_slot(uint32_t g, const FxPlanArgs &a, const PlanOneShared &sh, uint32_t &sidx)
+template <int NT> __device__ __forceinline__ uint32_t plan_one_slot(uint32_t g, const FxPlanArgs &a, const PlanOneShared<NT> &sh, uint32_t &sidx)
 {
     if (a.nstreams <= PLAN_LDS_STREAMS) { sidx = plan_stream_of(sh.sbase, a.nstreams, g); return sh.cbase[sidx] + (g - sh.sbase[sidx]); }
     sidx = plan_stream_of(a.stream_base, a.nstreams, g);
     return a.streams[sidx].chain_base + (g - a.stream_base[sidx]);
 }
 
-extern "C" __global__ __launch_bounds__(PLAN_THREADS)
+template <int NT> __global__ __launch_bounds__(NT)
 void fx_planfused_kernel(const FxPlanArgs a)
 {
-    __shared__ PlanOneShared sh;
-    __shared__ uint4 keep[PLAN_KEEP * PLAN_THREADS];
-    constexpr uint32_t TILE = PLAN_KEEP * PLAN_THREADS;
+    constexpr uint32_t TILE = PLAN_TILE;
+    constexpr int KEEP = PLAN_TILE / NT, JB = PLAN_BATCH;
+    static_assert(NT % 64 == 0 && KEEP * NT == PLAN_TILE && KEEP % JB == 0, "whole waves; the tile is KEEP frames a thread, in whole batches");
+    __shared__ PlanOneShared<NT> sh;
+    __shared__ uint4 keep[PLAN_TILE];
     const PlanCounts<false> cnt{ sh.cnt + PO_CLS, sh.cnt + PO_DEC, sh.cnt + PO_VBC };
     const uint32_t tid = threadIdx.x, nstreams = a.nstreams;
 #ifdef FX_STAMPS
@@ -2031,7 +2051,7 @@
 #endif
     {
         const uint32_t *src = reinterpret_cast<const uint32_t *>(a.hdr); uint32_t *dst = reinterpret_cast<uint32_t *>(&sh.h);
-        for (int i = (int)tid; i < (int)(sizeof(FxBlockHdr) / 4); i += PLAN_THREADS) dst[i] = src[i];
+        for (int i = (int)tid; i < (int)(sizeof(FxBlockHdr) / 4); i += NT) dst[i] = src[i];
         if (tid < PO_N) { sh.cnt[tid] = 0u; sh.fill[tid] = 0u; }
         if (tid <= FX_PLL_CLASSES) sh.cls_base[tid] = 0u;
         if (tid < 8) sh.vbc_base[tid] = 0u;
@@ -2039,106 +2059,107 @@
     uint32_t N;
     if (nstreams <= PLAN_LDS_STREAMS) {
         uint32_t v[PLAN_NV] = { tid < nstreams ? a.chain_count[tid] : 0u, 0, 0, 0, 0, 0, 0 }, tot[PLAN_NV];
-        if (nstreams > 1) plan_scan(v, tot, sh.ws); else { tot[0] = v[0]; v[0] = 0u; }
+        if (nstreams > 1) plan_scan<NT>(v, tot, sh.ws); else { tot[0] = v[0]; v[0] = 0u; }
         if (tid < nstreams) { sh.sbase[tid] = v[0]; a.stream_base[tid] = v[0]; sh.cbase[tid] = a.streams[tid].chain_base; }
         if (tid == 0) { sh.sbase[nstreams] = tot[0]; a.stream_base[nstreams] = tot[0]; }
         __syncthreads();
         N = sh.sbase[nstreams];
-    } else N = plan_stream_bases(a.chain_count, nstreams, a.stream_base, sh.ws);
+    } else N = plan_stream_bases<NT>(a.chain_count, nstreams, a.stream_base, sh.ws);
 
     uint32_t run[PLAN_NV] = { 0, 0, 0, 0, 0, 0, 0 };
     for (int pass = N > TILE ? 0 : 1; pass < 2; pass++) {
 #pragma unroll
         for (int q = 0; q < PLAN_NV; q++) run[q] = 0u;
         for (uint32_t t0 = 0; t0 < N; t0 += TILE) {
-            const uint32_t nt = min(TILE, N - t0), t1 = t0 + nt, per = (nt + PLAN_THREADS - 1) / PLAN_THREADS, f0 = t0 + tid * per;
-            uint32_t st[PLAN_NV], tot[PLAN_NV];
-            uint32_t info[PLAN_KEEP];
+            const uint32_t nt = min(TILE, N - t0), t1 = t0 + nt, per = (nt + NT - 1) / NT, f0 = t0 + tid * per;
+            uint32_t st[PLAN_NV];
+            PlanWords w[KEEP]; uint32_t slot[KEEP], sidx[KEEP];
+#pragma unroll
+            for (int i = 0; i < KEEP; i++) {
+                const bool live = (uint32_t)i < per && f0 + i < t1;
+                slot[i] = plan_one_slot(live ? f0 + i : t0, a, sh, sidx[i]);
+                w[i] = plan_words(a.chain + slot[i]);
+            }
+#pragma unroll
+            for (int q = 0; q < PLAN_NV; q++) st[q] = 0u;
+#pragma unroll
+            for (int i = 0; i < KEEP; i++) {
+                uint32_t v[PLAN_NV];
+                (void)plan_sizes(w[i], (uint32_t)i < per && f0 + i < t1, a.detect, a.vb_blk, v);
+#pragma unroll
+                for (int q = 0; q < PLAN_NV; q++) st[q] += v[q];
+            }
             {
-                PlanWords w[PLAN_KEEP];
-#pragma unroll
-                for (int i = 0; i < PLAN_KEEP; i++) {
-                    const bool live = (uint32_t)i < per && f0 + i < t1;
-                    uint32_t sidx;
-                    w[i] = plan_words(a.chain + plan_one_slot(live ? f0 + i : t0, a, sh, sidx));
-                }
-#pragma unroll
-                for (int q = 0; q < PLAN_NV; q++) st[q] = 0u;
-#pragma unroll
-                for (int i = 0; i < PLAN_KEEP; i++) {
+                uint32_t tot[PLAN_NV];
+                plan_scan<NT>(st, tot, sh.ws);
+#pragma unroll
+                for (int q = 0; q < PLAN_NV; q++) { st[q] += run[q]; run[q] += tot[q]; }
+            }
+            if (pass == 0 || N <= TILE) {
+                uint32_t vb = st[PV_VB];
+#pragma unroll
+                for (int i = 0; i < KEEP; i++) {
                     uint32_t v[PLAN_NV];
                     const PlanFrame f = plan_sizes(w[i], (uint32_t)i < per && f0 + i < t1, a.detect, a.vb_blk, v);
-                    info[i] = f.valid ? f.vnb | plan_key(w[i].ms, w[i].fec0, w[i].fec1).pack() << 16 | 1u << 24 | (f.batch ? 1u << 25 : 0u) : 0u;
-#pragma unroll
-                    for (int q = 0; q < PLAN_NV; q++) st[q] += v[q];
-                }
-            }
-            plan_scan(st, tot, sh.ws);
-#pragma unroll
-            for (int q = 0; q < PLAN_NV; q++) st[q] += run[q];
-            if (pass == 0 || N <= TILE) {
-                uint32_t vb = st[PV_VB];
-#pragma unroll
-                for (int i = 0; i < PLAN_KEEP; i++) {
-                    const uint32_t vnb = info[i] & 0xffffu;
-                    const bool batch = ((info[i] >> 25) & 1u) && !plan_demote(vb, vnb, a.vb_cap);
-                    vb += vnb;
-                    if ((info[i] >> 24) & 1u) {
-                        const PlanKey key = PlanKey::unpack(info[i] >> 16);
+                    const bool batch = f.batch && !plan_demote(vb, f.vnb, a.vb_cap);
+                    vb += f.vnb;
+                    if (f.valid) {
+                        const PlanKey key = plan_key(w[i].ms, w[i].fec0, w[i].fec1);
                         atomicAdd(&sh.cnt[PO_CLS + key.cls], 1u);
                         atomicAdd(&sh.cnt[PO_DEC + key.dec(batch)], 1u);
-                        if (batch) atomicAdd(&sh.cnt[PO_VBC + key.vc], vnb);
+                        if (batch) atomicAdd(&sh.cnt[PO_VBC + key.vc], f.vnb);
                     }
                 }
             }
-            if (pass == 0) {
-#pragma unroll
-                for (int q = 0; q < PLAN_NV; q++) run[q] += tot[q];
-                continue;
-            }
+            if (pass == 0) continue;
             if (t0 == 0) {
                 __syncthreads();
                 if (tid == 0) plan_class_bases(cnt, sh.cls_base, sh.vbc_base);
                 __syncthreads();
             }
             PLAN_TICK(st1_);
-            for (uint32_t i = 0; i < per && f0 + i < t1; i++) {
-                const uint32_t g = f0 + i;
-                uint32_t sidx, v[PLAN_NV];
-                const uint32_t slot = plan_one_slot(g, a, sh, sidx);
-                const FxFrame *fp = a.chain + slot;
-                const PlanWords w = plan_words(fp);
-                PlanFrame f = plan_sizes(w, true, a.detect, a.vb_blk, v);
-                f.fp = fp; f.sidx = sidx;
-                if (f.batch && plan_demote(st[PV_VB], f.vnb, a.vb_cap)) { f.batch = false; f.vnb = 0; }
-                uint32_t at = 0;
-                if (f.valid) {
-                    const PlanKey key = plan_key(w.ms, w.fec0, w.fec1);
-                    const uint32_t pp = sh.cls_base[key.cls] + atomicAdd(&sh.fill[PO_CLS + key.cls], 1u);
-                    if (pp < a.list_cap) a.pll_list[pp] = g;
-                    const uint32_t rs = key.dec(f.batch), dp = atomicAdd(&sh.fill[PO_DEC + rs], 1u);
-                    if (dp < a.list_cap) a.dec_list[(size_t)rs * a.list_cap + dp] = g;
-                    if (f.batch) at = sh.vbc_base[key.vc] + atomicAdd(&sh.fill[PO_VBC + key.vc], f.vnb);
+#pragma unroll
+            for (int b0 = 0; b0 < KEEP; b0 += JB) {
+                if ((uint32_t)b0 >= per) break;
+                PlanRest r[JB];
+#pragma unroll
+                for (int i = 0; i < JB; i++) r[i] = plan_rest(a.chain + slot[b0 + i], a.streams + sidx[b0 + i]);
+#pragma unroll
+                for (int i = 0; i < JB; i++) {
+                    const uint32_t g = f0 + b0 + i;
+                    if ((uint32_t)(b0 + i) >= per || g >= t1) break;
+                    const PlanWords &wi = w[b0 + i];
+                    uint32_t v[PLAN_NV];
+                    PlanFrame f = plan_sizes(wi, true, a.detect, a.vb_blk, v);
+                    f.fp = a.chain + slot[b0 + i]; f.sidx = sidx[b0 + i];
+                    if (f.batch && plan_demote(st[PV_VB], f.vnb, a.vb_cap)) { f.batch = false; f.vnb = 0; }
+                    uint32_t at = 0;
+                    if (f.valid) {
+                        const PlanKey key = plan_key(wi.ms, wi.fec0, wi.fec1);
+                        const uint32_t pp = sh.cls_base[key.cls] + atomicAdd(&sh.fill[PO_CLS + key.cls], 1u);
+                        if (pp < a.list_cap) a.pll_list[pp] = g;
+                        const uint32_t rs = key.dec(f.batch), dp = atomicAdd(&sh.fill[PO_DEC + rs], 1u);
+                        if (dp < a.list_cap) a.dec_list[(size_t)rs * a.list_cap + dp] = g;
+                        if (f.batch) at = sh.vbc_base[key.vc] + atomicAdd(&sh.fill[PO_VBC + key.vc], f.vnb);
+                    }
+                    keep[g - t0] = make_uint4(at, f.vnb, st[PV_MF], f.nblk);
+                    plan_emit(a.pjobs + g, a.recs + g, r[i], wi, f, st, a.eq, slot[b0 + i], at);
+#pragma unroll
+                    for (int q = 0; q < PLAN_NV; q++) st[q] += v[q];
                 }
-                keep[g - t0] = make_uint4(at, f.vnb, st[PV_MF], f.nblk);
-                plan_emit(a.pjobs + g, a.recs + g, fp, a.streams + sidx, w, f, st, a.eq, slot, at);
-#pragma unroll
-                for (int q = 0; q < PLAN_NV; q++) st[q] += v[q];
             }
             __syncthreads();
             PLAN_TICK(st2_);
-            for (uint32_t k = tid >> 4; k < nt; k += PLAN_THREADS / 16) {
+            for (uint32_t k = tid >> 4; k < nt; k += NT / 16) {
                 const uint4 kp = keep[k];
                 const uint32_t g = t0 + k, sub = tid & 15u;
                 for (uint32_t b = sub; b < kp.y; b += 16u) if (kp.x + b < a.vb_cap) { a.vb_items[kp.x + b] = g; a.vb_items[a.vb_cap + kp.x + b] = b; }
                 for (uint32_t c = sub; c < kp.w; c += 16u) if (kp.z + c < a.mf_cap) { a.mf_job[kp.z + c] = g; a.mf_c0[kp.z + c] = c * 1024u; }
             }
-#pragma unroll
-            for (int q = 0; q < PLAN_NV; q++) run[q] += tot[q];
             __syncthreads();
         }
     }
-    plan_pad_lists(cnt, sh.cls_base, sh.vbc_base, a);
+    plan_pad_lists<NT>(cnt, sh.cls_base, sh.vbc_base, a);
     PLAN_TICK(st6_);
     __threadfence(); __syncthreads();
     PLAN_TICK(st7_);
@@ -2149,14 +2170,17 @@
         plan_fill_hdr(sh.h, N, run, cnt, sh.cls_base, sh.vbc_base, a);
     }
     __syncthreads();
-    plan_mirror_hdr(sh.h, a);
-}
-
-extern "C" hipError_t fx_launch_plan(hipStream_t st, unsigned grid, int fused, const FxPlanArgs &a)
+    plan_mirror_hdr<NT>(sh.h, a);
+}
+
+extern "C" hipError_t fx_launch_plan(hipStream_t st, unsigned grid, int fused, unsigned threads, const FxPlanArgs &a)
 {
     const unsigned g = grid < 1u ? 1u : (grid > PLAN_MAXG ? PLAN_MAXG : grid);
-    if (fused && g == 1u) hipLaunchKernelGGL(fx_planfused_kernel, dim3(1), dim3(PLAN_THREADS), 0, st, a);
-    else {
+    if (fused && g == 1u) {
+        if (threads == 512u) hipLaunchKernelGGL((fx_planfused_kernel<512>), dim3(1), dim3(512), 0, st, a);
+        else if (threads == 256u) hipLaunchKernelGGL((fx_planfused_kernel<256>), dim3(1), dim3(256), 0, st, a);
+        else return hipErrorInvalidValue;
+    } else {
         hipLaunchKernelGGL(fx_plan_kernel, dim3(g), dim3(PLAN_THREADS), 0, st, a);
         hipLaunchKernelGGL(fx_planlists_kernel, dim3(g), dim3(PLAN_THREADS), 0, st, a);
     }
diff --git a/gr-liquiddsp_amd/csrc/fx_launch.h b/gr-liquiddsp_amd/csrc/fx_launch.h
--- a/gr-liquiddsp_amd/csrc/fx_launch.h
+++ b/gr-liquiddsp_amd/csrc/fx_launch.h
@@ -20,7 +20,7 @@
 extern "C" hipError_t fx_launch_chainfast(unsigned nstreams, hipStream_t st, const FxStreamDesc *streams, const FxWalkJob *jobs, const FxWalkResult *results,
                                           const FxFrame *frames, FxFrame *chain, uint32_t *chain_count, FxBlockHdr *hdr, uint32_t force_repair,
                                           FxWalkJob *jobs_rw, uint32_t *req_list, uint32_t *stat, uint32_t pass);
-extern "C" hipError_t fx_launch_plan(hipStream_t st, unsigned grid, int fused, const FxPlanArgs &a);
+extern "C" hipError_t fx_launch_plan(hipStream_t st, unsigned grid, int fused, unsigned threads, const FxPlanArgs &a);
 extern "C" unsigned fx_plan_ws_words(void);
 extern "C" hipError_t fx_launch_vbpre(const FxVbpreGang *gang, hipStream_t st, const FxTables *T, int clean_on, int early_tail);
 extern "C" hipError_t fx_launch_vbitems(unsigned first_item, unsigned n_items, hipStream_t st, const FxPayJob *jobs, const uint32_t *vb_items, uint32_t item_cap,
```

Result: faster. 40440 Msamples/s, median of 6 (+6.6%).
